# cvxgrp/DNLP

Measured on NVIDIA B200. Metric: oracle evals/s (f, grad f, g, J, Hess L), higher is better.
Workload: dtype f64

## Files before the change

dnlp_b200/_cabi.py:

```python
import ctypes as C
import os

import numpy as np

from . import tape as T

_PKG = os.path.dirname(os.path.abspath(__file__))
LIB_PATH = os.path.join(_PKG, "libdnlp_b200.so")

PROG_IDS = {"f": 0, "grad": 1, "g": 2, "jac": 3, "hess": 4, "all": 5}
NPROG = 6

c_i64p = C.POINTER(C.c_int64)
c_i32p = C.POINTER(C.c_int32)
c_f64p = C.POINTER(C.c_double)
c_f32p = C.POINTER(C.c_float)


class InstrDesc(C.Structure):
    _fields_ = [
        ("kind", C.c_int32), ("dst_space", C.c_int32), ("dst_off", C.c_int64), ("count", C.c_int64),
        ("fcode", C.c_int32), ("a_stride", C.c_int32), ("b_stride", C.c_int32), ("accumulate", C.c_int32),
        ("param", C.c_double), ("a_off", C.c_int64), ("b_off", C.c_int64),
        ("ptr", c_i64p), ("coef", c_f64p), ("f1", c_i32p), ("f2", c_i32p), ("pos", c_i32p),
        ("nterms", C.c_int64), ("row_len", C.c_int32), ("uses_lam", C.c_int32),
        ("level", C.c_int32), ("dep_mask", C.c_int32),
        ("Q", c_f64p), ("ncols", C.c_int64), ("x_off", C.c_int64), ("alpha", C.c_double),
        ("s_slot", C.c_int64),
        ("deps", c_i32p), ("n_deps", C.c_int64),
        ("dst_stride", C.c_int32), ("reserved0", C.c_int32), ("post_scale", C.c_double), ("qpos", c_i32p),
    ]


class TapeDesc(C.Structure):
    _fields_ = [
        ("n", C.c_int64), ("m", C.c_int64), ("nslots", C.c_int64), ("nnz_jac", C.c_int64), ("nnz_hess", C.c_int64),
        ("n_instr", C.c_int32), ("instrs", C.POINTER(InstrDesc)),
        ("prog", c_i32p * NPROG), ("prog_len", C.c_int32 * NPROG),
        ("f_const", C.c_double), ("grad_const", c_f64p), ("g_const", c_f64p),
        ("jac_const", c_f64p), ("hess_const", c_f64p),
        ("n_params", C.c_int64), ("params", c_f64p),
    ]


EXPORTS = [
    "dnlp_device_count", "dnlp_version", "dnlp_device_synchronize", "dnlp_create", "dnlp_destroy", "dnlp_last_error",
    "dnlp_eval_f", "dnlp_eval_grad", "dnlp_eval_g", "dnlp_eval_jac", "dnlp_eval_hess", "dnlp_eval_all",
    "dnlp_host_alloc", "dnlp_host_free", "dnlp_upload_point", "dnlp_run_device", "dnlp_profile_instrs",
    "dnlp_read_output", "dnlp_kernel_launches", "dnlp_set_cache", "dnlp_set_graphs", "dnlp_set_parallel", "dnlp_set_windows", "dnlp_set_dynamic", "dnlp_eval_dyn", "dnlp_bind_outputs", "dnlp_set_params", "dnlp_instr_kernel", "dnlp_run", "dnlp_output_ptr",
    "dnlp_batch_create", "dnlp_batch_destroy", "dnlp_batch_last_error", "dnlp_batch_eval", "dnlp_batch_upload",
    "dnlp_batch_run_device", "dnlp_batch_read_output", "dnlp_batch_profile_instrs", "dnlp_batch_kernel_launches", "dnlp_batch_profile_groups",
    "dnlp_batch_kkt_setup", "dnlp_batch_kkt_solve", "dnlp_batch_kkt_matrix",
    "dnlp_comm_unique_id", "dnlp_comm_create", "dnlp_comm_destroy", "dnlp_comm_last_error", "dnlp_comm_has_nccl",
    "dnlp_comm_ipc_handle", "dnlp_comm_open_peers", "dnlp_comm_allreduce_host",
    "dnlp_shard_create", "dnlp_shard_destroy", "dnlp_shard_last_error", "dnlp_shard_set_output",
    "dnlp_shard_root_handles", "dnlp_shard_open_root", "dnlp_shard_eval", "dnlp_shard_run_device", "dnlp_shard_set_layout",
    "dnlp_shard_share_control", "dnlp_shard_share_output", "dnlp_shard_share_unlink", "dnlp_shard_share_release", "dnlp_shard_share_reset",
    "dnlp_shard_share_inputs", "dnlp_shard_post_command", "dnlp_shard_wait_command",
]

_lib = None


def lib():
    global _lib
    if _lib is not None:
        return _lib
    if not os.path.exists(LIB_PATH):
        raise RuntimeError(
            "dnlp_b200: %s is missing - build it with `python -m dnlp_b200.build` "
            "(there is no CPU fallback for the oracle)" % LIB_PATH)
    L = C.CDLL(LIB_PATH)
    vp = C.c_void_p
    L.dnlp_device_count.restype = C.c_int
    L.dnlp_version.restype = C.c_char_p
    L.dnlp_device_synchronize.argtypes = [C.c_int]
    L.dnlp_create.argtypes = [C.POINTER(TapeDesc), C.c_int, C.POINTER(vp)]
    L.dnlp_destroy.argtypes = [vp]
    L.dnlp_destroy.restype = None
    L.dnlp_last_error.argtypes = [vp]
    L.dnlp_last_error.restype = C.c_char_p
    L.dnlp_eval_f.argtypes = [vp, c_f64p, c_f64p]
    L.dnlp_eval_grad.argtypes = [vp, c_f64p, c_f64p]
    L.dnlp_eval_g.argtypes = [vp, c_f64p, c_f64p]
    L.dnlp_eval_jac.argtypes = [vp, c_f64p, c_f64p]
    L.dnlp_eval_hess.argtypes = [vp, c_f64p, c_f64p, C.c_double, c_f64p]
    L.dnlp_eval_all.argtypes = [vp, c_f64p, c_f64p, C.c_double] + [c_f64p] * 5
    L.dnlp_host_alloc.argtypes = [C.c_int64]
    L.dnlp_host_alloc.restype = vp
    L.dnlp_host_free.argtypes = [vp]
    L.dnlp_host_free.restype = None
    L.dnlp_upload_point.argtypes = [vp, c_f64p, c_f64p, C.c_double]
    L.dnlp_run_device.argtypes = [vp, C.c_int32, C.c_int32, c_f32p]
    L.dnlp_profile_instrs.argtypes = [vp, C.c_int32, C.c_int32, c_f32p]
    L.dnlp_read_output.argtypes = [vp, C.c_int32, c_f64p]
    L.dnlp_kernel_launches.argtypes = [vp]
    L.dnlp_kernel_launches.restype = C.c_int64
    L.dnlp_set_cache.argtypes = [vp, C.c_int32]
    L.dnlp_set_graphs.argtypes = [vp, C.c_int32]
    L.dnlp_set_parallel.argtypes = [vp, C.c_int32]
    L.dnlp_set_windows.argtypes = [vp, C.c_int32]
    L.dnlp_run.argtypes = [vp, C.c_int32, c_f64p, c_f64p, C.c_double]
    L.dnlp_output_ptr.argtypes = [vp, C.c_int32]
    L.dnlp_output_ptr.restype = vp
    L.dnlp_instr_kernel.argtypes = [vp, C.c_int32]
    L.dnlp_instr_kernel.restype = C.c_char_p
    L.dnlp_set_params.argtypes = [vp, c_f64p, C.c_int64]
    L.dnlp_bind_outputs.argtypes = [vp, c_f64p, c_f64p, c_f64p, c_f64p, C.c_int32]
    L.dnlp_set_dynamic.argtypes = [vp, C.c_int32, c_i32p, C.c_int64]
    L.dnlp_eval_dyn.argtypes = [vp, C.c_int32, c_f64p, c_f64p, C.c_double, c_f64p]
    L.dnlp_batch_create.argtypes = [C.POINTER(TapeDesc), C.c_int, C.c_int32, C.POINTER(vp)]
    L.dnlp_batch_destroy.argtypes = [vp]
    L.dnlp_batch_destroy.restype = None
    L.dnlp_batch_last_error.argtypes = [vp]
    L.dnlp_batch_last_error.restype = C.c_char_p
    L.dnlp_batch_eval.argtypes = [vp] + [c_f64p] * 8
    L.dnlp_batch_upload.argtypes = [vp, c_f64p, c_f64p, c_f64p]
    L.dnlp_batch_run_device.argtypes = [vp, C.c_int32, C.c_int32, c_f32p]
    L.dnlp_batch_read_output.argtypes = [vp, C.c_int32, c_f64p]
    L.dnlp_batch_profile_instrs.argtypes = [vp, C.c_int32, C.c_int32, c_f32p]
    L.dnlp_batch_profile_groups.argtypes = [vp, C.c_int32, c_f32p, c_f64p, C.c_int32]
    L.dnlp_batch_kernel_launches.argtypes = [vp]
    L.dnlp_batch_kernel_launches.restype = C.c_int64
    L.dnlp_batch_kkt_setup.argtypes = [vp, C.c_int64] + [c_i32p] * 5
    L.dnlp_batch_kkt_solve.argtypes = [vp, C.c_int32, c_i32p] + [c_f64p] * 5 + [c_i32p, c_f64p, c_f32p]
    L.dnlp_batch_kkt_matrix.argtypes = [vp, C.c_int32, c_f64p]
    cp = C.c_char_p
    L.dnlp_comm_unique_id.argtypes = [cp]
    L.dnlp_comm_create.argtypes = [cp, C.c_int, C.c_int, C.c_int, C.POINTER(vp)]
    L.dnlp_comm_destroy.argtypes = [vp]
    L.dnlp_comm_destroy.restype = None
    L.dnlp_comm_last_error.argtypes = [vp]
    L.dnlp_comm_last_error.restype = C.c_char_p
    L.dnlp_comm_has_nccl.argtypes = [vp]
    L.dnlp_comm_ipc_handle.argtypes = [vp, cp]
    L.dnlp_comm_open_peers.argtypes = [vp, cp]
    L.dnlp_comm_allreduce_host.argtypes = [vp, c_f64p, C.c_int64]
    L.dnlp_shard_create.argtypes = [vp, vp, C.c_int, C.POINTER(vp)]
    L.dnlp_shard_destroy.argtypes = [vp]
    L.dnlp_shard_destroy.restype = None
    L.dnlp_shard_last_error.argtypes = [vp]
    L.dnlp_shard_last_error.restype = C.c_char_p
    L.dnlp_shard_set_output.argtypes = [vp, C.c_int32, C.c_int64, c_i32p, c_i32p, C.c_int64, c_i32p, c_i32p,
                                        C.c_int64, c_f64p, C.c_int64, c_i32p]
    L.dnlp_shard_root_handles.argtypes = [vp, cp]
    L.dnlp_shard_open_root.argtypes = [vp, cp]
    L.dnlp_shard_set_layout.argtypes = [vp, C.c_int32, c_i64p, c_i64p, C.c_int32, c_i64p, c_i64p]
    L.dnlp_shard_eval.argtypes = [vp, C.c_int32, c_f64p, c_f64p, C.c_double, c_f64p]
    L.dnlp_shard_run_device.argtypes = [vp, C.c_int32, C.c_int32, c_f32p]
    L.dnlp_shard_share_control.argtypes = [vp, C.c_char_p, C.c_int32]
    L.dnlp_shard_share_output.argtypes = [vp, C.c_int32, C.c_char_p, C.c_int32, C.c_int64, c_i64p, c_i64p, c_i64p,
                                          C.POINTER(c_f64p)]
    L.dnlp_shard_share_unlink.argtypes = [C.c_char_p]
    L.dnlp_shard_share_release.argtypes = [C.c_void_p, C.c_int64]
    L.dnlp_shard_share_reset.argtypes = [vp]
    L.dnlp_shard_share_inputs.argtypes = [vp, C.c_char_p, C.c_char_p, C.c_int32, C.c_int64, C.c_int64,
                                          C.POINTER(c_f64p), C.POINTER(c_f64p)]
    L.dnlp_shard_post_command.argtypes = [vp, C.c_int32, c_f64p, c_f64p, C.c_double, C.c_int32, C.POINTER(C.c_int32)]
    L.dnlp_shard_wait_command.argtypes = [vp, C.c_double, C.POINTER(C.c_int32), C.POINTER(C.c_double),
                                          C.POINTER(C.c_int32)]
    _lib = L
    return L


def device_count():
    return int(lib().dnlp_device_count())


def device_synchronize(device=0):
    if lib().dnlp_device_synchronize(int(device)) != 0:
        raise RuntimeError("dnlp_b200: cudaDeviceSynchronize failed on device %d" % device)


def _p(arr, typ):
    return None if arr is None else arr.ctypes.data_as(typ)


def f64(a):
    return np.ascontiguousarray(a, dtype=np.float64)


def pinned_empty(count):
    L = lib()
    nbytes = max(int(count), 1) * 8
    ptr = L.dnlp_host_alloc(nbytes)
    if not ptr:
        raise MemoryError("cudaMallocHost(%d) failed" % nbytes)
    buf = (C.c_double * max(int(count), 1)).from_address(ptr)
    handle = _PinnedHandle(ptr)
    buf._dnlp_handle = handle
    arr = np.frombuffer(buf, dtype=np.float64, count=int(count))
    return arr, handle


def shared_view(addr, count):
    buf = (C.c_double * max(int(count), 1)).from_address(addr)
    buf._dnlp_handle = _SharedHandle(addr, int(count))
    return np.frombuffer(buf, dtype=np.float64, count=int(count))


class _SharedHandle:
    def __init__(self, addr, count):
        self.addr, self.count = addr, count

    def __del__(self):
        try:
            if self.addr:
                lib().dnlp_shard_share_release(self.addr, self.count)
                self.addr = None
        except Exception:
            pass


class _PinnedHandle:
    def __init__(self, ptr):
        self.ptr = ptr

    def free(self):
        """Kept for API compatibility: release happens when the last array view is collected."""

    def __del__(self):
        try:
            if self.ptr:
                lib().dnlp_host_free(self.ptr)
                self.ptr = None
        except Exception:
            pass


def make_tape_desc(tape):
    keep = []
    n_instr = len(tape.instrs)
    i32max = int(np.iinfo(np.int32).max)
    for what, v in (("value slots", tape.nslots), ("Jacobian entries", tape.jac_rows.size),
                    ("Hessian entries", tape.hess_rows.size)):
        if int(v) > i32max:
            raise OverflowError("dnlp_b200: %d %s exceed the int32 index range of the device tape" % (int(v), what))
    arr = (InstrDesc * max(n_instr, 1))()
    for i, ins in enumerate(tape.instrs):
        d = arr[i]
        d.kind, d.dst_space, d.dst_off, d.count = ins.kind, ins.dst_space, int(ins.dst_off), int(ins.count)
        d.fcode, d.a_stride, d.b_stride = int(ins.fcode), int(ins.a_stride), int(ins.b_stride)
        d.accumulate = int(bool(ins.accumulate))
        d.param, d.a_off, d.b_off = float(ins.param), int(ins.a_off), int(ins.b_off)
        d.uses_lam = int(bool(ins.uses_lam))
        d.level = int(ins.level)
        d.dep_mask = int(ins.dep_mask)
        d.alpha, d.ncols, d.x_off, d.s_slot = float(ins.alpha), int(ins.ncols), int(ins.x_off), int(ins.s_slot)
        d.dst_stride, d.post_scale = int(ins.dst_stride), float(ins.post_scale)
        if ins.kind == T.K_SPMVJ:
            qpos = np.ascontiguousarray(ins.qpos, dtype=np.int32)
            keep.append(qpos)
            d.qpos = _p(qpos, c_i32p)
        if ins.kind in (T.K_POLY, T.K_SPMVJ):
            lens = np.diff(ins.ptr)
            uniform = lens.size > 0 and bool(np.all(lens == lens[0])) and lens[0] >= 1
            coef = f64(ins.coef)
            f1 = np.ascontiguousarray(ins.f1, dtype=np.int32)
            has_f2 = bool(np.any(ins.f2 >= 0))
            f2 = np.ascontiguousarray(ins.f2, dtype=np.int32) if has_f2 else None
            ptr = None if uniform else np.ascontiguousarray(ins.ptr, dtype=np.int64)
            keep += [coef, f1, f2, ptr]
            d.ptr, d.coef, d.f1, d.f2 = _p(ptr, c_i64p), _p(coef, c_f64p), _p(f1, c_i32p), _p(f2, c_i32p)
            d.nterms = int(coef.size)
            d.row_len = int(lens[0]) if uniform else 0
        elif ins.kind == T.K_GEMV:
            Q = f64(ins.Q)
            keep.append(Q)
            d.Q = _p(Q, c_f64p)
        elif ins.kind == T.K_SCALE:
            coef = f64(ins.coef)
            keep.append(coef)
            d.coef = _p(coef, c_f64p)
        if len(ins.deps):
            deps = np.ascontiguousarray(sorted(ins.deps), dtype=np.int32)
            keep.append(deps)
            d.deps, d.n_deps = _p(deps, c_i32p), int(deps.size)
        if ins.pos is not None:
            pos = np.ascontiguousarray(ins.pos, dtype=np.int32)
            keep.append(pos)
            d.pos = _p(pos, c_i32p)
    td = TapeDesc()
    td.n, td.m, td.nslots = tape.n, tape.m, tape.nslots
    td.nnz_jac, td.nnz_hess = int(tape.jac_rows.size), int(tape.hess_rows.size)
    td.n_instr, td.instrs = n_instr, arr
    for name, pid in PROG_IDS.items():
        p = np.ascontiguousarray(tape.programs.get(name, []), dtype=np.int32)
        keep.append(p)
        td.prog[pid] = _p(p, c_i32p) if p.size else None
        td.prog_len[pid] = int(p.size)
    consts = [f64(tape.grad_const), f64(tape.g_const), f64(tape.jac_const), f64(tape.hess_const)]
    keep += consts
    td.f_const = float(tape.f_const)
    td.grad_const, td.g_const, td.jac_const, td.hess_const = [_p(c, c_f64p) if c.size else None for c in consts]
    pv = f64(getattr(tape, "param_values", np.zeros(0)))
    keep.append(pv)
    td.n_params = int(getattr(tape, "n_params", 0))
    if pv.size != td.n_params:
        raise ValueError("tape has %d parameter slots but %d values" % (td.n_params, pv.size))
    td.params = _p(pv, c_f64p) if pv.size else None
    keep += [arr, td]
    return td, keep


def _require_device(L):
    if L.dnlp_device_count() <= 0:
        raise RuntimeError("dnlp_b200: no CUDA device visible (the oracle has no CPU fallback)")


class DeviceTape:

    def __init__(self, tape, device=0):
        L = lib()
        _require_device(L)
        self.tape = tape
        td, keep = make_tape_desc(tape)
        h = C.c_void_p()
        if L.dnlp_create(C.byref(td), int(device), C.byref(h)) != 0:
            raise RuntimeError("dnlp_create failed: %s" % L.dnlp_last_error(None).decode())
        self.h = h
        self._L = L

    def check(self, rc):
        if rc != 0:
            if not self.h:
                raise RuntimeError("dnlp_b200: oracle closed")
            raise RuntimeError("dnlp_b200: %s" % self._L.dnlp_last_error(self.h).decode())

    def set_params(self, values):
        self.check(self._L.dnlp_set_params(self.h, values.ctypes.data_as(c_f64p), int(values.size)))

    def bind_outputs(self, f, grad, g, jac, eager):
        p = lambda a: a.ctypes.data_as(c_f64p)
        self.check(self._L.dnlp_bind_outputs(self.h, p(f), p(grad), p(g), p(jac), int(bool(eager))))

    def close(self):
        if getattr(self, "h", None):
            self._L.dnlp_destroy(self.h)
            self.h = None

    def __del__(self):
        try:
            self.close()
        except Exception:
            pass


class DeviceBatch:

    def __init__(self, tape, batch, device=0):
        L = lib()
        _require_device(L)
        self.tape, self.batch = tape, int(batch)
        td, keep = make_tape_desc(tape)
        h = C.c_void_p()
        if L.dnlp_batch_create(C.byref(td), int(device), int(batch), C.byref(h)) != 0:
            raise RuntimeError("dnlp_batch_create failed: %s" % L.dnlp_batch_last_error(None).decode())
        self.h = h
        self._L = L

    def check(self, rc):
        if rc != 0:
            if not self.h:
                raise RuntimeError("dnlp_b200: oracle closed")
            raise RuntimeError("dnlp_b200: %s" % self._L.dnlp_batch_last_error(self.h).decode())

    def close(self):
        if getattr(self, "h", None):
            self._L.dnlp_batch_destroy(self.h)
            self.h = None

    def __del__(self):
        try:
            self.close()
        except Exception:
            pass
```

dnlp_b200/csrc/dnlp_cabi.cu:

```cuda
#include "dnlp_engine.h"

#include <algorithm>
#include <cstdio>
#include <cstdlib>
#include <cstring>
#include <string>
#include <thread>
#include <unordered_map>
#include <vector>

namespace {
thread_local std::string g_create_error;
}

namespace {

using namespace dnlp;

template <int F, bool B>
void launch_elem_t(const dnlp_oracle *o, const dnlp_instr_desc &d, int grid) {
  elem_kernel<F, B><<<grid, 256, 0, o->cur>>>(o->V, d.a_off, d.a_stride, d.b_off, d.b_stride,
                                                d.dst_off, d.count, d.param, d.dst_stride > 0 ? d.dst_stride : 1,
                                                d.post_scale);
}

bool launch_elem(const dnlp_oracle *o, const dnlp_instr_desc &d, int grid) {
  switch (d.fcode) {
#define U(F) case F: launch_elem_t<F, false>(o, d, grid); return true;
#define Bn(F) case F: launch_elem_t<F, true>(o, d, grid); return true;
    U(F_EXP) U(F_LOG) U(F_ENTR) U(F_NEG_LOG_M1) U(F_RECIP) U(F_NEG_RECIP) U(F_NEG_RECIP_SQ)
    U(F_LOGISTIC) U(F_LOGISTIC_D1) U(F_LOGISTIC_D2) U(F_POW)
    U(F_SIN) U(F_COS) U(F_NEG_SIN) U(F_NEG_COS) U(F_TAN) U(F_TAN_D1) U(F_TAN_D2)
    U(F_SINH) U(F_COSH) U(F_TANH) U(F_TANH_D1) U(F_TANH_D2)
    U(F_ASINH) U(F_ASINH_D1) U(F_ASINH_D2) U(F_ATANH) U(F_ATANH_D1) U(F_ATANH_D2)
    U(F_XEXP) U(F_XEXP_D1) U(F_XEXP_D2)
    Bn(F_REL_ENTR) Bn(F_LOG_RATIO_P1) Bn(F_DIV) Bn(F_DIV_SQ) Bn(F_DIV_CUBE)
#undef U
#undef Bn
    default: return false;
  }
}

template <int G>
void launch_poly_g(const dnlp_oracle *o, const DevInstr &I, double *dst, int grid) {
  const dnlp_instr_desc &d = I.d;
  const bool uni = d.ptr == nullptr;
#define LP(H, Un)                                                                                   \
  poly_rows_kernel<G, 2, H, Un><<<grid, 256, 0, o->cur>>>(o->V, dst, d.ptr, d.row_len, d.coef,   \
                                                             d.f1, d.f2, d.pos, d.count, d.accumulate)
  if (I.has_f2) { if (uni) LP(true, true); else LP(true, false); }
  else { if (uni) LP(false, true); else LP(false, false); }
#undef LP
}

void choose_window(const int32_t *f1, const int32_t *f2, int64_t nterms, int64_t nslots, int *w0, int *W) {
  *w0 = -1; *W = 0;
  constexpr int BK = 256;
  const int64_t nb = nslots / BK + 1;
  std::vector<int64_t> cnt((size_t)nb + 1, 0);
  int64_t total = 0;
  for (int64_t t = 0; t < nterms; ++t) {
    if (f1[t] >= 0) { ++cnt[f1[t] / BK]; ++total; }
    if (f2 && f2[t] >= 0) { ++cnt[f2[t] / BK]; ++total; }
  }
  if (total == 0) return;
  const int widths[3] = {17, 33, 65};
  int64_t best[3], at[3];
  for (int w = 0; w < 3; ++w) {
    const int64_t Wb = widths[w] < nb ? widths[w] : nb;
    int64_t run = 0;
    for (int64_t b = 0; b < Wb; ++b) run += cnt[b];
    best[w] = run; at[w] = 0;
    for (int64_t b = Wb; b < nb; ++b) {
      run += cnt[b] - cnt[b - Wb];
      if (run > best[w]) { best[w] = run; at[w] = b - Wb + 1; }
    }
  }
  if (2 * best[2] < total) return;
  for (int w = 0; w < 3; ++w) {
    if (10 * best[w] >= 9 * best[2]) {
      const int64_t Wb = widths[w] < nb ? widths[w] : nb;
      int64_t lo = at[w] * BK, hi = lo + Wb * BK;
      if (hi > nslots) hi = nslots;
      *w0 = (int)lo; *W = (int)(hi - lo);
      return;
    }
  }
}

}

int dnlp_oracle::launch(DevInstr &I) {
  const dnlp_instr_desc &d = I.d;
  if (d.count <= 0) return 0;
  double *dst = (d.dst_space == DNLP_DST_V) ? V + d.dst_off : out[d.dst_space] + d.dst_off;
  if (cur == nullptr) { cur = stream; cur_lane = 0; }
  switch (d.kind) {
    case DNLP_ELEM: {
      int grid = grid_for((d.count + 1) / 2, 1);
      if (!launch_elem(this, d, grid)) { err = "unknown elementwise function code"; return 1; }
      if (I.kname.empty()) I.kname = "elem_kernel<" + std::to_string(d.fcode) + ", " + (d.fcode >= 40 ? "1" : "0") + ">";
      break;
    }
    case DNLP_POLY: {
      if (I.contig && I.const_coef && d.count == 1 && d.nterms >= 2048 && !d.pos) {
        int64_t blocks = (d.nterms + 256 * 4 - 1) / (256 * 4);
        int64_t cap = (int64_t)sm_count * 4;
        int grid = (int)(blocks < cap ? blocks : cap);
        if (I.has_f2)
          sum_range_kernel<true><<<grid, 256, 0, cur>>>(V, dst, I.s0, I.s1, d.nterms, I.c0, d.accumulate, scratch + cur_lane * 4096, ticket + cur_lane * 16);
        else
          sum_range_kernel<false><<<grid, 256, 0, cur>>>(V, dst, I.s0, I.s1, d.nterms, I.c0, d.accumulate, scratch + cur_lane * 4096, ticket + cur_lane * 16);
        if (I.kname.empty()) I.kname = std::string("sum_range_kernel<") + (I.has_f2 ? "1" : "0") + ">";
        break;
      }
      if (I.contig && d.ptr == nullptr && d.row_len == 1 && !d.pos && !d.accumulate && d.count >= 4096) {
        int grid = grid_for(d.count, 1);
        if (I.has_f2)
          poly1_contig_kernel<true><<<grid, 256, 0, cur>>>(V, dst, d.coef, I.s0, I.s1, d.count);
        else
          poly1_contig_kernel<false><<<grid, 256, 0, cur>>>(V, dst, d.coef, I.s0, I.s1, d.count);
        if (I.kname.empty()) I.kname = std::string("poly1_contig_kernel<") + (I.has_f2 ? "1" : "0") + ">";
        break;
      }
      if (d.count == 1 && d.nterms >= 2048 && !d.pos) {
        int64_t blocks = (d.nterms + 256 * 4 - 1) / (256 * 4);
        int64_t cap = (int64_t)sm_count * 4;
        int grid = (int)(blocks < cap ? blocks : cap);
        if (I.has_f2)
          poly_reduce_kernel<true><<<grid, 256, 0, cur>>>(V, dst, d.coef, d.f1, d.f2, d.nterms, d.accumulate, scratch + cur_lane * 4096, ticket + cur_lane * 16);
        else
          poly_reduce_kernel<false><<<grid, 256, 0, cur>>>(V, dst, d.coef, d.f1, d.f2, d.nterms, d.accumulate, scratch + cur_lane * 4096, ticket + cur_lane * 16);
        if (I.kname.empty()) I.kname = std::string("poly_reduce_kernel<") + (I.has_f2 ? "1" : "0") + ">";
        break;
      }
      if (d.ptr == nullptr && d.row_len == 1) {
        int grid = grid_for((d.count + 3) / 4, 1);
        if (grid > sm_count * poly1_grid_mult) grid = sm_count * poly1_grid_mult;
        if (I.has_f2)
          poly1_stream_kernel<4, true><<<grid, 256, 0, cur>>>(V, dst, d.coef, d.f1, d.f2, d.pos, d.count, d.accumulate);
        else
          poly1_stream_kernel<4, false><<<grid, 256, 0, cur>>>(V, dst, d.coef, d.f1, d.f2, d.pos, d.count, d.accumulate);
        if (I.kname.empty()) I.kname = std::string("poly1_stream_kernel<4, ") + (I.has_f2 ? "1" : "0") + ">";
        break;
      }
      if (I.flat && flat_enabled) {
        const bool win = I.winW > 0 && win_enabled && I.winW <= 33 * 256;
        const size_t smem = win ? (size_t)I.winW * sizeof(double) : 0;
        const int per_sm = smem > 36 * 1024 ? 2 : 4;
        const int64_t nchunks = I.nchunks;
        const int64_t need = (nchunks + dnlp::FLAT_WARPS - 1) / dnlp::FLAT_WARPS;
        const int grid = (int)(need < (int64_t)sm_count * per_sm ? need : (int64_t)sm_count * per_sm);
#define LF(H, Wn, Pd)                                                                                      \
        poly_flat_kernel<H, Wn, Pd><<<grid, 256, smem, cur>>>(V, dst, d.ptr, d.row_len, d.coef, d.f1, d.f2,    \
                                                              d.pos, d.nterms, d.accumulate, I.chunk_row0,    \
                                                              I.chunk_term0, nchunks, I.win0,                 \
                                                              win ? I.winW : 0, I.pad_shift)
        const bool pad = I.pad_shift < 31;
        if (I.has_f2) {
          if (win) { if (pad) LF(true, true, true); else LF(true, true, false); }
          else { if (pad) LF(true, false, true); else LF(true, false, false); }
        } else {
          if (win) { if (pad) LF(false, true, true); else LF(false, true, false); }
          else { if (pad) LF(false, false, true); else LF(false, false, false); }
        }
#undef LF
        if (I.kname.empty())
          I.kname = std::string("poly_flat_kernel<") + (I.has_f2 ? "1" : "0") + ", " + (win ? "1" : "0") + ", " +
                    (pad ? "1" : "0") + ">";
        break;
      }
      int G = 1;
      while (G < 32 && (double)(2 * G) <= 0.8 * I.mean_len) G <<= 1;
      int grid = grid_for((d.count + 1) / 2, G);
      switch (G) {
        case 1: launch_poly_g<1>(this, I, dst, grid); break;
        case 2: launch_poly_g<2>(this, I, dst, grid); break;
        case 4: launch_poly_g<4>(this, I, dst, grid); break;
        case 8: launch_poly_g<8>(this, I, dst, grid); break;
        case 16: launch_poly_g<16>(this, I, dst, grid); break;
        default: launch_poly_g<32>(this, I, dst, grid); break;
      }
      if (I.kname.empty())
        I.kname = "poly_rows_kernel<" + std::to_string(G) + ", 2, " + (I.has_f2 ? "1" : "0") + ", " +
                  (d.ptr == nullptr ? "1" : "0") + ">";
      break;
    }
    case DNLP_SPMVJ: {
      double *jac = out[DNLP_DST_JAC];
      if (I.flat && flat_enabled) {
        const int64_t need = (I.nchunks + dnlp::FLAT_WARPS - 1) / dnlp::FLAT_WARPS;
        const int grid = (int)(need < (int64_t)sm_count * 3 ? need : (int64_t)sm_count * 3);
        if (I.pad_shift < 31)
          spmvj_flat_kernel<true><<<grid, 256, 0, cur>>>(V, dst, jac, d.ptr, d.row_len, d.coef, d.f1, I.jrank, I.jsorted, d.pos,
                                                         d.nterms, I.chunk_row0, I.chunk_term0, I.nchunks, I.pad_shift);
        else
          spmvj_flat_kernel<false><<<grid, 256, 0, cur>>>(V, dst, jac, d.ptr, d.row_len, d.coef, d.f1, I.jrank, I.jsorted, d.pos,
                                                          d.nterms, I.chunk_row0, I.chunk_term0, I.nchunks, I.pad_shift);
        if (I.kname.empty()) I.kname = std::string("spmvj_flat_kernel<") + (I.pad_shift < 31 ? "1" : "0") + ">";
      } else {
        spmvj_rows_kernel<<<grid_for(d.count, 1), 256, 0, cur>>>(V, dst, jac, d.ptr, d.row_len, d.coef, d.f1, d.qpos, d.pos, d.count);
        if (I.kname.empty()) I.kname = "spmvj_rows_kernel";
      }
      break;
    }
    case DNLP_GEMV: {
      size_t smem = (size_t)d.ncols * sizeof(double);
      if ((d.ncols & 1) == 0 && smem <= 96 * 1024) {
        int64_t cap = (int64_t)sm_count * 2;
        int grid = (int)(d.count < cap ? d.count : cap);
        gemv_cta_kernel<4, 16><<<grid, 512, smem, cur>>>(d.Q, V, d.x_off, dst, d.count, d.ncols, d.alpha);
        if (I.kname.empty()) I.kname = "gemv_cta_kernel<4, 16>";
      } else {
        int in_smem = smem <= 96 * 1024 ? 1 : 0;
        if (!in_smem) smem = 0;
        int64_t blocks = (d.count + 7) / 8;
        int64_t cap = (int64_t)sm_count * (in_smem && smem > 48 * 1024 ? 2 : 4);
        int grid = (int)(blocks < cap ? (blocks < 1 ? 1 : blocks) : cap);
        dnlp_gemv_rows_kernel<8><<<grid, 256, smem, cur>>>(d.Q, V, d.x_off, dst, d.count, d.ncols, d.alpha, in_smem);
        if (I.kname.empty()) I.kname = "dnlp_gemv_rows_kernel<8>";
      }
      break;
    }
    case DNLP_SCALE: {
      int grid = grid_for((d.count + 1) / 2, 1);
      if (!d.pos && !d.accumulate && ((reinterpret_cast<uintptr_t>(d.coef) | reinterpret_cast<uintptr_t>(dst)) & 15) == 0)
        { scale_stream_kernel<4><<<sm_count * 16, 256, 0, cur>>>(V, d.s_slot, d.coef, dst, d.count);
          if (I.kname.empty()) I.kname = "scale_stream_kernel<4>"; }
      else
        scale_kernel<<<grid, 256, 0, cur>>>(V, d.s_slot, d.coef, dst, d.pos, d.count, d.accumulate);
      break;
    }
    default:
      err = "unknown instruction kind";
      return 1;
  }
  ++launches;
  cudaError_t e = cudaPeekAtLastError();
  if (e != cudaSuccess) {
    err = std::string("kernel launch failed: ") + cudaGetErrorString(e);
    return 1;
  }
  return 0;
}

int dnlp_oracle::build_batches() {
  for (int bi = 0; bi < 2 * DNLP_NPROG; ++bi) {
    const int p = bi >> 1;
    const bool want_short = (bi & 1) != 0;
    ElemBatch &B = batch[bi];
    std::vector<dnlp::ElemDesc> descs;
    for (int32_t id : prog[p]) {
      const dnlp_instr_desc &d = instrs[id].d;
      if (d.kind != DNLP_ELEM || d.level != 0 || d.uses_lam || d.dst_space != DNLP_DST_V || d.count <= 0) continue;
      if ((d.count < batch_split) != want_short) continue;
      bool merged = false;
      for (auto &e : descs) {
        if (e.nout < 3 && e.a_off == d.a_off && e.b_off == d.b_off && e.count == d.count &&
            e.a_stride == d.a_stride && e.b_stride == d.b_stride) {
          e.fcode[e.nout] = d.fcode; e.param[e.nout] = d.param; e.dst_off[e.nout] = d.dst_off;
          e.dst_stride[e.nout] = d.dst_stride > 0 ? d.dst_stride : 1; e.scale[e.nout] = d.post_scale; ++e.nout;
          merged = true;
          break;
        }
      }
      if (!merged) {
        dnlp::ElemDesc e{};
        e.a_off = d.a_off; e.b_off = d.b_off; e.count = d.count; e.a_stride = d.a_stride; e.b_stride = d.b_stride;
        e.nout = 1; e.fcode[0] = d.fcode; e.param[0] = d.param; e.dst_off[0] = d.dst_off;
        e.dst_stride[0] = d.dst_stride > 0 ? d.dst_stride : 1; e.scale[0] = d.post_scale;
        for (int k = 1; k < 3; ++k) { e.dst_stride[k] = 1; e.scale[k] = 1.0; }
        descs.push_back(e);
      }
      B.members.push_back(id);
    }
    if (B.members.size() < 2) { B.members.clear(); continue; }
    for (auto &e : descs) {
      e.group = dnlp::GRP_NONE;
      if (e.nout < 2 || !fuse_enabled) continue;
      const int fam = dnlp::elem_family(e.fcode[0]);
      bool same = fam != dnlp::GRP_NONE;
      for (int k = 1; k < e.nout; ++k) same = same && dnlp::elem_family(e.fcode[k]) == fam;
      if (same) e.group = fam;
    }
    int64_t tiles = 0;
    for (auto &e : descs) { e.tile0 = tiles; tiles += (e.count + dnlp::ELEM_TILE - 1) / dnlp::ELEM_TILE; }
    B.ndesc = (int)descs.size();
    B.total_tiles = tiles;
    if (upload(descs.data(), (int64_t)descs.size(), &B.descs)) return 1;
  }
  return 0;
}

int dnlp_oracle::launch_node(int32_t node) {
  if (node >= 0) return launch(instrs[node]);
  ElemBatch &B = batch[-node - 1];
  if (cur == nullptr) { cur = stream; cur_lane = 0; }
  int64_t cap = (int64_t)sm_count * 8;
  int grid = (int)(B.total_tiles < cap ? B.total_tiles : cap);
  dnlp::elem_batch_kernel<<<grid, 256, 0, cur>>>(V, B.descs, B.ndesc, B.total_tiles);
  ++launches;
  cudaError_t e = cudaPeekAtLastError();
  if (e != cudaSuccess) { err = std::string("kernel launch failed: ") + cudaGetErrorString(e); return 1; }
  return 0;
}

int dnlp_oracle::issue_serial(const std::vector<int32_t> &nodes) {
  cur = stream; cur_lane = 0;
  for (int32_t nd : nodes) if (launch_node(nd)) return 1;
  return 0;
}

cudaEvent_t dnlp_oracle::event_at(size_t i) {
  while (ev_pool.size() <= i) {
    cudaEvent_t e = nullptr;
    if (cudaEventCreateWithFlags(&e, cudaEventDisableTiming) != cudaSuccess) return nullptr;
    ev_pool.push_back(e);
  }
  return ev_pool[i];
}

int dnlp_oracle::issue_parallel(const std::vector<int32_t> &nodes) {
  const size_t N = nodes.size();
  if (N < 2 || !parallel_enabled) return issue_serial(nodes);
  std::unordered_map<int32_t, int> producer;
  for (size_t k = 0; k < N; ++k) {
    if (nodes[k] >= 0) producer[nodes[k]] = (int)k;
    else for (int32_t id : batch[-nodes[k] - 1].members) producer[id] = (int)k;
  }
  std::vector<int> lane_of(N, 0);
  int last_on_lane[NLANE];
  bool joined[NLANE];
  for (int l = 0; l < NLANE; ++l) { last_on_lane[l] = -1; joined[l] = (l == 0); }
  int last_writer[6] = {-1, -1, -1, -1, -1, -1};
  int rr = 0;
  cudaEvent_t fork = event_at(0);
  if (!fork) { err = "cudaEventCreate failed"; return 1; }
  CK(cudaEventRecord(fork, stream));
  std::vector<int> deps;
  for (size_t k = 0; k < N; ++k) {
    deps.clear();
    if (nodes[k] >= 0) {
      const DevInstr &I = instrs[nodes[k]];
      for (int32_t d : I.deps) {
        auto it = producer.find(d);
        if (it != producer.end() && it->second < (int)k) deps.push_back(it->second);
      }
      if (I.d.dst_space != DNLP_DST_V) {
        if (last_writer[I.d.dst_space] >= 0) deps.push_back(last_writer[I.d.dst_space]);
        last_writer[I.d.dst_space] = (int)k;
      }
      if (I.d.kind == DNLP_SPMVJ) {
        if (last_writer[DNLP_DST_JAC] >= 0) deps.push_back(last_writer[DNLP_DST_JAC]);
        last_writer[DNLP_DST_JAC] = (int)k;
      }
    }
    int L = -1;
    if (nodes[k] >= 0 && big_serial_terms > 0 && instrs[nodes[k]].d.kind != DNLP_ELEM &&
        instrs[nodes[k]].d.nterms >= big_serial_terms) L = 0;
    if (L < 0) for (int d : deps) if (last_on_lane[lane_of[d]] == d && !(big_serial_terms > 0 && lane_of[d] == 0)) { L = lane_of[d]; break; }
    if (L < 0) for (int l = big_serial_terms > 0 ? 1 : 0; l < NLANE; ++l) if (last_on_lane[l] < 0) { L = l; break; }
    if (L < 0) { L = big_serial_terms > 0 ? 1 + rr % (NLANE - 1) : rr; rr = (rr + 1) % NLANE; }
    if (!joined[L]) { CK(cudaStreamWaitEvent(lane[L], fork, 0)); joined[L] = true; }
    for (int d : deps)
      if (lane_of[d] != L) CK(cudaStreamWaitEvent(lane[L], event_at(1 + (size_t)d), 0));
    cur = lane[L]; cur_lane = L;
    const int rc = launch_node(nodes[k]);
    cur = stream; cur_lane = 0;
    if (rc) return 1;
    cudaEvent_t done = event_at(1 + k);
    if (!done) { err = "cudaEventCreate failed"; return 1; }
    CK(cudaEventRecord(done, lane[L]));
    lane_of[k] = L;
    last_on_lane[L] = (int)k;
  }
  for (int l = 1; l < NLANE; ++l)
    if (joined[l] && last_on_lane[l] >= 0) CK(cudaStreamWaitEvent(stream, event_at(1 + (size_t)last_on_lane[l]), 0));
  return 0;
}

int dnlp_oracle::run_programs(const int *progs, int nprogs, bool force) {
  std::vector<int32_t> nodes;
  std::vector<uint8_t> done(valid);
  if (force || !cache_enabled) std::fill(done.begin(), done.end(), 0);
  uint64_t key = 1469598103934665603ull;
  for (int q = 0; q < nprogs; ++q) {
    const int p = progs[q];
    for (int bi = 2 * p + 1; bi >= 2 * p; --bi) {
      ElemBatch &B = batch[bi];
      bool use_batch = !B.members.empty();
      if (use_batch) for (int32_t id : B.members) if (done[id]) { use_batch = false; break; }
      if (use_batch) {
        nodes.push_back(-(bi + 1));
        key = (key ^ (uint64_t)(0x10000 + bi)) * 1099511628211ull;
        for (int32_t id : B.members) done[id] = 2;
      }
    }
    for (int32_t id : prog[p]) {
      const DevInstr &I = instrs[id];
      const bool keep = cacheable(I);
      if (done[id] == 2) continue;
      if (keep && done[id]) continue;
      nodes.push_back(id);
      key = (key ^ (uint64_t)(id + 1)) * 1099511628211ull;
      if (keep) done[id] = 1;
    }
    for (auto &f : done) if (f == 2) f = 1;
  }
  if (nodes.empty()) return 0;

  if (capturing) {
    if (issue_parallel(nodes)) return 1;
  } else if (graphs_enabled && nodes.size() >= 2) {
    auto it = graphs.find(key);
    if (it != graphs.end()) {
      const GraphEntry &ge = it->second;
      if (ge.plan == nodes) {
        CK(cudaGraphLaunch(ge.exec, stream));
        launches += ge.nlaunch;
      } else if (issue_serial(nodes)) return 1;
    } else if (graphs.size() < 64) {
      const int64_t before = launches;
      capturing = true;
      CK(cudaStreamBeginCapture(stream, cudaStreamCaptureModeThreadLocal));
      const int rc = issue_parallel(nodes);
      cudaGraph_t g = nullptr;
      cudaError_t ce = cudaStreamEndCapture(stream, &g);
      capturing = false;
      if (rc) { if (g) cudaGraphDestroy(g); cudaGetLastError(); return 1; }
      if (ce != cudaSuccess) { err = std::string("graph capture failed: ") + cudaGetErrorString(ce); return 1; }
      GraphEntry ge;
      ge.plan = nodes;
      ge.nlaunch = launches - before;
      CK(cudaGraphInstantiate(&ge.exec, g, 0));
      cudaGraphDestroy(g);
      graphs.emplace(key, ge);
      CK(cudaGraphLaunch(ge.exec, stream));
    } else if (issue_serial(nodes)) return 1;
  } else if (issue_serial(nodes)) return 1;

  for (int32_t nd : nodes) {
    if (nd < 0) { for (int32_t id : batch[-nd - 1].members) valid[id] = 1; continue; }
    if (cacheable(instrs[nd])) valid[nd] = 1;
  }
  return 0;
}

static int stage_threads() { return dnlp_stage_threads(); }
int dnlp_stage_threads() {
  static const int T = [] {
    unsigned hw = std::thread::hardware_concurrency();
    int ranks = 1;
    if (const char *e = getenv("LOCAL_WORLD_SIZE")) ranks = atoi(e) > 0 ? atoi(e) : 1;
    if (const char *e = getenv("DNLP_STAGE_THREADS")) return atoi(e) > 0 ? atoi(e) : 1;
    int t = (int)(hw / (unsigned)ranks) - (ranks > 1 ? 1 : 2);
    return t < 1 ? 1 : (t > 14 ? 14 : t);
  }();
  return T;
}

static bool stage_point(double *dst, const double *src, int64_t n, bool have_old) {
  const size_t bytes = (size_t)n * sizeof(double);
  auto work = [&](int64_t lo, int64_t hi, bool *changed) {
    const size_t b = (size_t)(hi - lo) * sizeof(double);
    if (have_old && memcmp(dst + lo, src + lo, b) == 0) { *changed = false; return; }
    memcpy(dst + lo, src + lo, b);
    *changed = true;
  };
  if (bytes < (4u << 20)) {
    bool ch = true;
    work(0, n, &ch);
    return ch;
  }
  const int T = stage_threads();
  const int64_t chunk = (n + T - 1) / T;
  int any = 0;
#pragma omp parallel for num_threads(T) schedule(static, 1) reduction(| : any)
  for (int t = 0; t < T; ++t) {
    const int64_t lo = t * chunk, hi = lo + chunk < n ? lo + chunk : n;
    if (lo < hi) {
      bool ch = true;
      work(lo, hi, &ch);
      any |= ch ? 1 : 0;
    }
  }
  return any != 0;
}

static bool same_as_mirror(const double *mir, const double *src, int64_t n) {
  const size_t bytes = (size_t)n * sizeof(double);
  if (bytes < (1u << 20)) return memcmp(mir, src, bytes) == 0;
  const int T = stage_threads();
  const int64_t chunk = (n + T - 1) / T;
  int diff = 0;
#pragma omp parallel for num_threads(T) schedule(static, 1) reduction(| : diff)
  for (int t = 0; t < T; ++t) {
    const int64_t lo = t * chunk, hi = lo + chunk < n ? lo + chunk : n;
    if (lo < hi && memcmp(mir + lo, src + lo, (size_t)(hi - lo) * sizeof(double)) != 0) diff |= 1;
  }
  return diff == 0;
}

static int stage_and_upload(double *hmir, double *dev, const double *src, int64_t count, bool have_old,
                            cudaStream_t stream, bool *changed, std::string &err) {
  *changed = false;
  if (have_old && count > 0 && same_as_mirror(hmir, src, count)) return 0;
  constexpr int64_t PIECE = (4 << 20) / sizeof(double);
  for (int64_t lo = 0; lo < count; lo += PIECE) {
    const int64_t len = count - lo < PIECE ? count - lo : PIECE;
    if (stage_point(hmir + lo, src + lo, len, have_old)) {
      CK(cudaMemcpyAsync(dev + lo, hmir + lo, (size_t)len * sizeof(double), cudaMemcpyHostToDevice, stream));
      *changed = true;
    }
  }
  return 0;
}

int dnlp_oracle::put_x(const double *x) {
  bool changed = false;
  if (stage_and_upload(hx, V, x, n, have_last_x && cache_enabled, stream, &changed, err)) return 1;
  if (!changed && have_last_x && cache_enabled) return 0;
  invalidate(1);
  have_last_x = true;
  ++x_epoch;
  return 0;
}

int dnlp_oracle::put_lam(const double *lam, double sigma) {
  if (!have_last_lam || hlam[0] != sigma) {
    invalidate(2);
    hlam[0] = sigma;
    CK(cudaMemcpyAsync(V + n, hlam, sizeof(double), cudaMemcpyHostToDevice, stream));
  }
  if (m > 0 && lam != nullptr) {
    bool lam_changed = false;
    if (stage_and_upload(hlam + 1, V + n + 1, lam, m, have_last_lam, stream, &lam_changed, err)) return 1;
    if (lam_changed) invalidate(4);
  }
  have_last_lam = true;
  return 0;
}

int dnlp_oracle::put_x_runs(const double *xg, const std::vector<int64_t> &src, const std::vector<int64_t> &len) {
  bool any = false;
  int64_t off = 0;
  for (size_t r = 0; r < src.size(); ++r) {
    bool ch = false;
    if (stage_and_upload(hx + off, V + off, xg + src[r], len[r], have_last_x && cache_enabled, stream, &ch, err)) return 1;
    any = any || ch;
    off += len[r];
  }
  if (off != n) { err = "variable runs do not cover the local point"; return 1; }
  if (!any && have_last_x && cache_enabled) return 0;
  invalidate(1);
  have_last_x = true;
  ++x_epoch;
  return 0;
}

int dnlp_oracle::put_lam_runs(const double *lg, double sigma, const std::vector<int64_t> &src, const std::vector<int64_t> &len) {
  if (!have_last_lam || hlam[0] != sigma) {
    invalidate(2);
    hlam[0] = sigma;
    CK(cudaMemcpyAsync(V + n, hlam, sizeof(double), cudaMemcpyHostToDevice, stream));
  }
  int64_t off = 0;
  bool any = false;
  if (lg == nullptr) { have_last_lam = true; return 0; }
  for (size_t r = 0; r < src.size(); ++r) {
    bool ch = false;
    if (stage_and_upload(hlam + 1 + off, V + n + 1 + off, lg + src[r], len[r], have_last_lam, stream, &ch, err)) return 1;
    any = any || ch;
    off += len[r];
  }
  if (off != m) { err = "constraint runs do not cover the local multipliers"; return 1; }
  if (any) invalidate(4);
  have_last_lam = true;
  return 0;
}

int dnlp_oracle::fetch(int space, double *host) {
  if (host == nullptr || out_len[space] == 0) return 0;
  CK(cudaMemcpyAsync(host, out[space], (size_t)out_len[space] * sizeof(double), cudaMemcpyDeviceToHost, stream));
  return 0;
}

int dnlp_oracle::launch_eager() {
  CK(cudaStreamWaitEvent(stream, ev_copied, 0));
  const int progs[4] = {DNLP_PROG_F, DNLP_PROG_GRAD, DNLP_PROG_G, DNLP_PROG_JAC};
  if (run_programs(progs, 4, false)) return 1;
  for (int s = DNLP_DST_GRAD; s <= DNLP_DST_JAC; ++s)
    if (bound[s] && dyn_len[s] > 0) {
      dnlp::gather_kernel<<<grid_for(dyn_len[s], 1), 256, 0, stream>>>(out[s], dyn_pos[s], dyn_buf[s], dyn_len[s]);
      ++launches;
    }
  CK(cudaEventRecord(ev_ready, stream));
  CK(cudaStreamWaitEvent(cstream, ev_ready, 0));
  for (int s = DNLP_DST_F; s <= DNLP_DST_JAC; ++s) {
    if (!bound[s]) continue;
    const bool dyn = s != DNLP_DST_F && dyn_len[s] > 0;
    const int64_t cnt = dyn ? dyn_len[s] : out_len[s];
    if (cnt > 0)
      CK(cudaMemcpyAsync(bound[s], dyn ? dyn_buf[s] : out[s], (size_t)cnt * sizeof(double), cudaMemcpyDeviceToHost, cstream));
    CK(cudaEventRecord(ev_out[s], cstream));
  }
  CK(cudaEventRecord(ev_copied, cstream));
  eager_epoch = x_epoch;
  return 0;
}

int dnlp_oracle::deliver(int space, int prog, double *host_out) {
  if (eager && cache_enabled && host_out != nullptr && bound[space] == host_out) {
    if (eager_epoch != x_epoch && launch_eager()) return 1;
    CK(cudaEventSynchronize(ev_out[space]));
    return 0;
  }
  if (eager) CK(cudaStreamWaitEvent(stream, ev_copied, 0));
  if (run_program(prog, false)) return 1;
  if (fetch(space, host_out)) return 1;
  CK(cudaStreamSynchronize(stream));
  return 0;
}

extern "C" {

int dnlp_device_count(void) {
  int c = 0;
  if (cudaGetDeviceCount(&c) != cudaSuccess) { cudaGetLastError(); return 0; }
  return c;
}

const char *dnlp_version(void) { return "dnlp_b200 0.2 (sm_100a)"; }

int dnlp_device_synchronize(int device) {
  if (cudaSetDevice(device) != cudaSuccess || cudaDeviceSynchronize() != cudaSuccess) { cudaGetLastError(); return 1; }
  return 0;
}

const char *dnlp_last_error(dnlp_oracle *o) { return o ? o->err.c_str() : g_create_error.c_str(); }

void dnlp_destroy(dnlp_oracle *o) {
  if (!o) return;
  cudaSetDevice(o->device);
  if (o->stream) cudaStreamSynchronize(o->stream);
  for (auto &kv : o->graphs) if (kv.second.exec) cudaGraphExecDestroy(kv.second.exec);
  for (void *p : o->owned) cudaFree(p);
  if (o->hx) cudaFreeHost(o->hx);
  if (o->hlam) cudaFreeHost(o->hlam);
  if (o->cstream) cudaStreamSynchronize(o->cstream);
  if (o->ev0) cudaEventDestroy(o->ev0);
  if (o->ev1) cudaEventDestroy(o->ev1);
  if (o->ev_ready) cudaEventDestroy(o->ev_ready);
  if (o->ev_copied) cudaEventDestroy(o->ev_copied);
  for (int s2 = 0; s2 < 6; ++s2) if (o->ev_out[s2]) cudaEventDestroy(o->ev_out[s2]);
  if (o->cstream) cudaStreamDestroy(o->cstream);
  for (cudaEvent_t e : o->ev_pool) cudaEventDestroy(e);
  for (int l = 1; l < dnlp_oracle::NLANE; ++l) if (o->lane[l]) cudaStreamDestroy(o->lane[l]);
  if (o->stream) cudaStreamDestroy(o->stream);
  delete o;
}

static int create_impl(dnlp_oracle *o, const dnlp_tape_desc *t) {
  std::string &err = o->err;
  CK(cudaSetDevice(o->device));
  cudaDeviceProp prop;
  CK(cudaGetDeviceProperties(&prop, o->device));
  o->sm_count = prop.multiProcessorCount;
  CK(cudaStreamCreateWithFlags(&o->stream, cudaStreamNonBlocking));
  CK(cudaEventCreate(&o->ev0));
  CK(cudaEventCreate(&o->ev1));
  CK(cudaStreamCreateWithFlags(&o->cstream, cudaStreamNonBlocking));
  CK(cudaEventCreateWithFlags(&o->ev_ready, cudaEventDisableTiming));
  CK(cudaEventCreateWithFlags(&o->ev_copied, cudaEventDisableTiming));
  for (int s2 = 0; s2 < 6; ++s2) CK(cudaEventCreateWithFlags(&o->ev_out[s2], cudaEventDisableTiming));
  o->n = t->n; o->m = t->m; o->nslots = t->nslots; o->nnz_jac = t->nnz_jac; o->nnz_hess = t->nnz_hess;
  o->n_params = t->n_params;
  if (t->n_params < 0 || t->n + 1 + t->m + t->n_params > t->nslots) { err = "parameter slots exceed the value buffer"; return 1; }
  if (const char *e = getenv("DNLP_WIN_MIN_TERMS")) o->win_min_terms = atoll(e);
  if (const char *e = getenv("DNLP_NO_SIGMA_CACHE")) o->sigma_cache_enabled = atoi(e) == 0;
  if (const char *e = getenv("DNLP_BATCH_SPLIT")) o->batch_split = atoll(e);
  if (const char *e = getenv("DNLP_FLAT_MIN_TERMS")) o->flat_min_terms = atoll(e);
  if (const char *e = getenv("DNLP_NO_FLAT")) o->flat_enabled = atoi(e) == 0;
  if (const char *e = getenv("DNLP_POLY1_GRID_MULT")) o->poly1_grid_mult = atoi(e) > 0 ? atoi(e) : 4;
  if (const char *e = getenv("DNLP_WINDOWS")) o->win_enabled = atoi(e) != 0;
  if (const char *e = getenv("DNLP_NO_WINDOWS")) o->win_enabled = atoi(e) == 0 && o->win_enabled;
  if (const char *e = getenv("DNLP_NO_ELEM_FUSION")) o->fuse_enabled = atoi(e) == 0;
  if (const char *e = getenv("DNLP_NO_PARALLEL")) o->parallel_enabled = atoi(e) == 0;
  if (const char *e = getenv("DNLP_BIG_SERIAL_TERMS")) o->big_serial_terms = atoll(e);

  void *p = nullptr;
  CK(cudaMalloc(&p, (size_t)(t->nslots + 2) * sizeof(double)));
  o->owned.push_back(p);
  o->V = static_cast<double *>(p);
  CK(cudaMemset(o->V, 0, (size_t)(t->nslots + 2) * sizeof(double)));
  if (t->n_params > 0 && t->params)
    CK(cudaMemcpy(o->V + t->n + 1 + t->m, t->params, (size_t)t->n_params * sizeof(double), cudaMemcpyHostToDevice));

  CK(cudaMallocHost(&p, (size_t)(t->n + 2) * sizeof(double)));
  o->hx = static_cast<double *>(p);
  CK(cudaMallocHost(&p, (size_t)(t->m + 2) * sizeof(double)));
  o->hlam = static_cast<double *>(p);
  CK(cudaMalloc(&p, (size_t)dnlp_oracle::NLANE * 4096 * sizeof(double)));
  o->owned.push_back(p);
  o->scratch = static_cast<double *>(p);
  CK(cudaMalloc(&p, (size_t)dnlp_oracle::NLANE * 16 * sizeof(unsigned int)));
  o->owned.push_back(p);
  o->ticket = static_cast<unsigned int *>(p);
  CK(cudaMemset(o->ticket, 0, (size_t)dnlp_oracle::NLANE * 16 * sizeof(unsigned int)));
  o->lane[0] = o->stream;
  for (int l = 1; l < dnlp_oracle::NLANE; ++l) CK(cudaStreamCreateWithFlags(&o->lane[l], cudaStreamNonBlocking));
  o->cur = o->stream;

  const int64_t lens[6] = {0, 1, t->n, t->m, t->nnz_jac, t->nnz_hess};
  const double *consts[6] = {nullptr, &t->f_const, t->grad_const, t->g_const, t->jac_const, t->hess_const};
  for (int s = 1; s < 6; ++s) {
    o->out_len[s] = lens[s];
    CK(cudaMalloc(&p, (size_t)(lens[s] + 2) * sizeof(double)));
    o->owned.push_back(p);
    o->out[s] = static_cast<double *>(p);
    if (lens[s] > 0) {
      if (consts[s])
        CK(cudaMemcpy(o->out[s], consts[s], (size_t)lens[s] * sizeof(double), cudaMemcpyHostToDevice));
      else
        CK(cudaMemset(o->out[s], 0, (size_t)lens[s] * sizeof(double)));
    }
  }

  o->instrs.resize(t->n_instr);
  o->valid.assign(t->n_instr, 0);
  for (int i = 0; i < t->n_instr; ++i) {
    const dnlp_instr_desc &h = t->instrs[i];
    DevInstr &D = o->instrs[i];
    D.d = h;
    D.d.ptr = nullptr; D.d.coef = nullptr; D.d.f1 = nullptr; D.d.f2 = nullptr; D.d.pos = nullptr; D.d.Q = nullptr;
    D.d.deps = nullptr;
    D.d.qpos = nullptr;
    if (D.d.dst_stride <= 0) D.d.dst_stride = 1;
    if (h.kind == DNLP_ELEM && D.d.post_scale == 0.0 && h.post_scale == 0.0) D.d.post_scale = 1.0;
    for (int64_t k = 0; k < h.n_deps; ++k) {
      if (h.deps[k] < 0 || h.deps[k] >= i) { err = "instruction depends on a later or unknown instruction"; return 1; }
      D.deps.push_back(h.deps[k]);
    }
    if (h.kind == DNLP_POLY || h.kind == DNLP_SPMVJ) {
      if (h.ptr) { if (o->upload(h.ptr, h.count + 1, const_cast<int64_t **>(&D.d.ptr))) return 1; }
      if (o->upload(h.coef, h.nterms, const_cast<double **>(&D.d.coef))) return 1;
      if (o->upload(h.f1, h.nterms, const_cast<int32_t **>(&D.d.f1))) return 1;
      if (h.f2) { if (o->upload(h.f2, h.nterms, const_cast<int32_t **>(&D.d.f2))) return 1; }
      if (h.kind == DNLP_SPMVJ) {
        if (h.f2 || !h.qpos) { err = "SPMVJ needs single-factor terms and Jacobian positions"; return 1; }
        for (int64_t t2 = 0; t2 < h.nterms; ++t2) {
          if (h.f1[t2] >= 0 && ((h.f1[t2] & 1) || h.f1[t2] + 1 >= t->nslots)) { err = "SPMVJ: value slots must be even (pair layout)"; return 1; }
          if (h.qpos[t2] >= t->nnz_jac) { err = "SPMVJ: Jacobian position out of range"; return 1; }
        }
        if (o->upload(h.qpos, h.nterms, const_cast<int32_t **>(&D.d.qpos))) return 1;
      }
      D.has_f2 = h.f2 != nullptr;
      D.mean_len = h.count > 0 ? (double)h.nterms / (double)h.count : 1.0;
      if (h.kind == DNLP_POLY && h.nterms >= 2048 && (h.count == 1 || (!h.ptr && h.row_len == 1)) && h.f1[0] >= 0 &&
          (!h.f2 || h.f2[0] >= 0)) {
        bool contig = true, cc = true;
        for (int64_t t2 = 1; t2 < h.nterms && contig; ++t2) {
          if (h.f1[t2] != h.f1[0] + t2) contig = false;
          else if (h.f2 && h.f2[t2] != h.f2[0] + t2) contig = false;
          if (h.coef[t2] != h.coef[0]) cc = false;
        }
        D.contig = contig;
        D.const_coef = contig && cc;
        D.s0 = h.f1[0];
        D.s1 = h.f2 ? h.f2[0] : 0;
        D.c0 = h.coef[0];
      }
      if (h.nterms >= o->flat_min_terms && h.count >= 2 && !(h.ptr == nullptr && h.row_len == 1) &&
          D.mean_len <= 64.0 && h.count < ((int64_t)1 << 31) - 1) {
        auto rb = [&](int64_t r) -> int64_t { return h.ptr ? h.ptr[r] : r * (int64_t)h.row_len; };
        std::vector<int32_t> row0;
        std::vector<int64_t> term0;
        bool ok = true;
        int64_t R = 0;
        while (R < h.count) {
          const int64_t a0 = rb(R) & ~(int64_t)1;
          int64_t Rn = R;
          while (Rn < h.count && rb(Rn + 1) <= a0 + dnlp::FLAT_CHUNK) ++Rn;
          if (Rn == R) { ok = false; break; }
          row0.push_back((int32_t)R);
          term0.push_back(a0);
          R = Rn;
        }
        if (ok) {
          row0.push_back((int32_t)h.count);
          D.nchunks = (int64_t)term0.size();
          if (o->upload(row0.data(), (int64_t)row0.size(), &D.chunk_row0)) return 1;
          if (o->upload(term0.data(), (int64_t)term0.size(), &D.chunk_term0)) return 1;
          const int64_t L = (int64_t)(D.mean_len + 0.5) > 0 ? (int64_t)(D.mean_len + 0.5) : 1;
          int best_conf = 1 << 30;
          const int shifts[3] = {31, 4, 5};
          for (int si = 0; si < 3; ++si) {
            int hits[16] = {0};
            int conf = 0;
            for (int j = 0; j < 16; ++j) {
              const int64_t k = j * L;
              const int64_t q = k + (shifts[si] >= 31 ? 0 : ((k >> shifts[si]) << 1));
              conf = std::max(conf, ++hits[q & 15]);
            }
            if (conf < best_conf) { best_conf = conf; D.pad_shift = shifts[si]; }
          }
          D.flat = true;
          if (h.kind == DNLP_SPMVJ) {
            std::vector<uint8_t> jrank((size_t)h.nterms + 2, 0);
            std::vector<int32_t> jsorted((size_t)h.nterms + 2, -1);
            const int64_t nch = D.nchunks;
#pragma omp parallel for schedule(static)
            for (int64_t ci = 0; ci < nch; ++ci) {
              const int64_t t0c = rb(row0[ci]), t1c = rb(row0[ci + 1]);
              const int nown = (int)(t1c - t0c);
              int idx[dnlp::FLAT_CHUNK];
              for (int i = 0; i < nown; ++i) idx[i] = i;
              std::sort(idx, idx + nown, [&](int a, int b) {
                const int32_t qa = h.qpos[t0c + a], qb = h.qpos[t0c + b];
                const uint32_t ua = qa < 0 ? 0xFFFFFFFFu : (uint32_t)qa, ub = qb < 0 ? 0xFFFFFFFFu : (uint32_t)qb;
                return ua != ub ? ua < ub : a < b;
              });
              for (int i = 0; i < nown; ++i) {
                jrank[t0c + idx[i]] = (uint8_t)i;
                jsorted[t0c + i] = h.qpos[t0c + idx[i]];
              }
            }
            if (o->upload(jrank.data(), (int64_t)jrank.size(), &D.jrank)) return 1;
            if (o->upload(jsorted.data(), (int64_t)jsorted.size(), &D.jsorted)) return 1;
          }
        }
      }
      if (D.flat && h.nterms >= o->win_min_terms)
        choose_window(h.f1, h.f2, h.nterms, t->nslots, &D.win0, &D.winW);
    } else if (h.kind == DNLP_GEMV) {
      if (o->upload(h.Q, h.count * h.ncols, const_cast<double **>(&D.d.Q))) return 1;
    } else if (h.kind == DNLP_SCALE) {
      if (o->upload(h.coef, h.count, const_cast<double **>(&D.d.coef))) return 1;
    }
    if ((h.kind == DNLP_POLY || h.kind == DNLP_SCALE || h.kind == DNLP_SPMVJ) && h.pos) {
      if (o->upload(h.pos, h.count, const_cast<int32_t **>(&D.d.pos))) return 1;
    }
  }
  for (const DevInstr &D : o->instrs)
    if (D.d.accumulate && D.d.dst_space >= 1 && D.d.dst_space <= 5) o->space_has_acc[D.d.dst_space] = true;
  for (int q = 0; q < DNLP_NPROG; ++q) {
    o->prog[q].assign(t->prog[q], t->prog[q] + t->prog_len[q]);
    for (int32_t id : o->prog[q])
      if (id < 0 || id >= t->n_instr) { err = "program references an unknown instruction"; return 1; }
  }
  if (o->build_batches()) return 1;
  CK(cudaFuncSetAttribute(dnlp::dnlp_gemv_rows_kernel<8>, cudaFuncAttributeMaxDynamicSharedMemorySize, 96 * 1024));
  CK(cudaFuncSetAttribute(dnlp::gemv_cta_kernel<4, 16>, cudaFuncAttributeMaxDynamicSharedMemorySize, 96 * 1024));
#define FA(H, Pd)                                                                                                       \
  CK(cudaFuncSetAttribute(dnlp::poly_flat_kernel<H, true, Pd>, cudaFuncAttributeMaxDynamicSharedMemorySize, 72 * 1024)); \
  CK(cudaFuncSetAttribute(dnlp::poly_flat_kernel<H, true, Pd>, cudaFuncAttributePreferredSharedMemoryCarveout, 100))
  FA(true, true); FA(true, false); FA(false, true); FA(false, false);
#undef FA
  CK(cudaStreamSynchronize(o->stream));
  return 0;
}

int dnlp_create(const dnlp_tape_desc *t, int device, dnlp_oracle **out) {
  *out = nullptr;
  dnlp_oracle *o = new dnlp_oracle();
  o->device = device;
  if (create_impl(o, t)) {
    g_create_error = o->err;
    dnlp_destroy(o);
    return 1;
  }
  *out = o;
  return 0;
}

#define ENTER(o)                                   \
  if ((o) == nullptr) { g_create_error = "oracle handle is NULL (closed or never created)"; return 1; } \
  std::string &err = (o)->err;                     \
  CK(cudaSetDevice((o)->device))

int dnlp_eval_f(dnlp_oracle *o, const double *x, double *f) {
  ENTER(o);
  if (o->put_x(x) || o->deliver(DNLP_DST_F, DNLP_PROG_F, f)) return 1;
  return 0;
}

int dnlp_eval_grad(dnlp_oracle *o, const double *x, double *grad) {
  ENTER(o);
  if (o->put_x(x) || o->deliver(DNLP_DST_GRAD, DNLP_PROG_GRAD, grad)) return 1;
  return 0;
}

int dnlp_eval_g(dnlp_oracle *o, const double *x, double *g) {
  ENTER(o);
  if (o->put_x(x) || o->deliver(DNLP_DST_G, DNLP_PROG_G, g)) return 1;
  return 0;
}

int dnlp_eval_jac(dnlp_oracle *o, const double *x, double *vals) {
  ENTER(o);
  if (o->put_x(x) || o->deliver(DNLP_DST_JAC, DNLP_PROG_JAC, vals)) return 1;
  return 0;
}

int dnlp_eval_hess(dnlp_oracle *o, const double *x, const double *lam, double sigma, double *vals) {
  ENTER(o);
  if (o->put_x(x) || o->put_lam(lam, sigma) || o->run_program(DNLP_PROG_HESS, false) ||
      o->fetch(DNLP_DST_HESS, vals)) return 1;
  CK(cudaStreamSynchronize(o->stream));
  return 0;
}

int dnlp_eval_all(dnlp_oracle *o, const double *x, const double *lam, double sigma,
                  double *f, double *grad, double *g, double *jac, double *hess) {
  ENTER(o);
  if (o->eager) CK(cudaStreamWaitEvent(o->stream, o->ev_copied, 0));
  if (o->put_x(x) || o->put_lam(lam, sigma) || o->run_program(DNLP_PROG_ALL, false)) return 1;
  if (o->fetch(DNLP_DST_F, f) || o->fetch(DNLP_DST_GRAD, grad) || o->fetch(DNLP_DST_G, g) ||
      o->fetch(DNLP_DST_JAC, jac) || o->fetch(DNLP_DST_HESS, hess)) return 1;
  CK(cudaStreamSynchronize(o->stream));
  return 0;
}

int dnlp_set_params(dnlp_oracle *o, const double *values, int64_t count) {
  ENTER(o);
  if (count != o->n_params) { err = "wrong number of parameter values"; return 1; }
  if (count == 0) return 0;
  CK(cudaStreamSynchronize(o->cstream));
  CK(cudaMemcpyAsync(o->V + o->n + 1 + o->m, values, (size_t)count * sizeof(double), cudaMemcpyHostToDevice, o->stream));
  CK(cudaStreamSynchronize(o->stream));
  o->invalidate(8);
  ++o->x_epoch;
  return 0;
}

int dnlp_bind_outputs(dnlp_oracle *o, double *f, double *grad, double *g, double *jac, int32_t eager) {
  ENTER(o);
  CK(cudaStreamSynchronize(o->cstream));
  o->bound[DNLP_DST_F] = f; o->bound[DNLP_DST_GRAD] = grad; o->bound[DNLP_DST_G] = g; o->bound[DNLP_DST_JAC] = jac;
  o->eager = eager != 0;
  o->eager_epoch = ~0ull;
  return 0;
}

int dnlp_set_dynamic(dnlp_oracle *o, int32_t space, const int32_t *pos, int64_t count) {
  ENTER(o);
  if (space < DNLP_DST_GRAD || space > DNLP_DST_HESS) { err = "bad output id"; return 1; }
  for (int64_t i = 0; i < count; ++i)
    if (pos[i] < 0 || pos[i] >= o->out_len[space]) { err = "dynamic position out of range"; return 1; }
  if (o->upload(pos, count, &o->dyn_pos[space])) return 1;
  void *p = nullptr;
  CK(cudaMalloc(&p, (size_t)(count + 2) * sizeof(double)));
  o->owned.push_back(p);
  o->dyn_buf[space] = static_cast<double *>(p);
  o->dyn_len[space] = count;
  return 0;
}

int dnlp_eval_dyn(dnlp_oracle *o, int32_t prog, const double *x, const double *lam, double sigma,
                  double *compact) {
  ENTER(o);
  if (prog < DNLP_PROG_GRAD || prog > DNLP_PROG_HESS) { err = "bad program id"; return 1; }
  const int space = prog + 1;
  if (o->put_x(x)) return 1;
  if (prog != DNLP_PROG_HESS && o->eager && o->cache_enabled && compact != nullptr && o->bound[space] == compact &&
      o->dyn_len[space] > 0) {
    if (o->eager_epoch != o->x_epoch && o->launch_eager()) return 1;
    CK(cudaEventSynchronize(o->ev_out[space]));
    return 0;
  }
  if (o->eager) CK(cudaStreamWaitEvent(o->stream, o->ev_copied, 0));
  if (prog == DNLP_PROG_HESS && o->put_lam(lam, sigma)) return 1;
  if (o->run_program(prog, false)) return 1;
  const int64_t cnt = o->dyn_len[space];
  if (cnt > 0) {
    int grid = o->grid_for(cnt, 1);
    dnlp::gather_kernel<<<grid, 256, 0, o->stream>>>(o->out[space], o->dyn_pos[space], o->dyn_buf[space], cnt);
    ++o->launches;
    CK(cudaMemcpyAsync(compact, o->dyn_buf[space], (size_t)cnt * sizeof(double), cudaMemcpyDeviceToHost, o->stream));
  }
  CK(cudaStreamSynchronize(o->stream));
  return 0;
}

int dnlp_run(dnlp_oracle *o, int32_t prog, const double *x, const double *lam, double sigma) {
  ENTER(o);
  if (o->cstream) CK(cudaStreamSynchronize(o->cstream));
  if (prog < 0 || prog >= DNLP_NPROG) { err = "bad program id"; return 1; }
  if (o->put_x(x)) return 1;
  if ((prog == DNLP_PROG_HESS || prog == DNLP_PROG_ALL) && o->put_lam(lam, sigma)) return 1;
  if (o->run_program(prog, false)) return 1;
  CK(cudaStreamSynchronize(o->stream));
  return 0;
}

void *dnlp_output_ptr(dnlp_oracle *o, int32_t space) {
  if (!o) return nullptr;
  if (space < DNLP_DST_F || space > DNLP_DST_HESS) return nullptr;
  return o->out[space];
}

void *dnlp_host_alloc(int64_t bytes) {
  void *p = nullptr;
  if (cudaMallocHost(&p, (size_t)bytes) != cudaSuccess) { cudaGetLastError(); return nullptr; }
  return p;
}

void dnlp_host_free(void *p) { if (p) cudaFreeHost(p); }

int dnlp_upload_point(dnlp_oracle *o, const double *x, const double *lam, double sigma) {
  ENTER(o);
  o->have_last_x = false;
  o->have_last_lam = false;
  if (o->put_x(x)) return 1;
  if (lam != nullptr || o->m == 0) { if (o->put_lam(lam, sigma)) return 1; }
  CK(cudaStreamSynchronize(o->stream));
  return 0;
}

int dnlp_run_device(dnlp_oracle *o, int32_t prog_mask, int32_t iters, float *elapsed_ms) {
  ENTER(o);
  if (o->cstream) CK(cudaStreamSynchronize(o->cstream));
  int progs[DNLP_NPROG], nprogs = 0;
  for (int p = 0; p < DNLP_NPROG; ++p) if (prog_mask & (1 << p)) progs[nprogs++] = p;
  if ((prog_mask & 0x1F) == 0x1F) { progs[0] = DNLP_PROG_ALL; nprogs = 1; }
  auto step = [&]() -> int {
    std::fill(o->valid.begin(), o->valid.end(), 0);
    return o->run_programs(progs, nprogs, false);
  };
  cudaGraphExec_t exec = nullptr;
  int64_t per_step = 0;
  if (iters <= 0) { if (elapsed_ms) *elapsed_ms = 0.f; return 0; }
  if (o->graphs_enabled) {
    const int64_t before = o->launches;
    o->capturing = true;
    CK(cudaStreamBeginCapture(o->stream, cudaStreamCaptureModeThreadLocal));
    const int rc = step();
    cudaGraph_t g = nullptr;
    cudaError_t ce = cudaStreamEndCapture(o->stream, &g);
    o->capturing = false;
    if (rc) { if (g) cudaGraphDestroy(g); return 1; }
    if (ce != cudaSuccess) { err = std::string("graph capture failed: ") + cudaGetErrorString(ce); return 1; }
    per_step = o->launches - before;
    o->launches = before;
    CK(cudaGraphInstantiate(&exec, g, 0));
    cudaGraphDestroy(g);
  }
  CK(cudaEventRecord(o->ev0, o->stream));
  for (int it = 0; it < iters; ++it) {
    if (exec) { CK(cudaGraphLaunch(exec, o->stream)); o->launches += per_step; }
    else if (step()) return 1;
  }
  CK(cudaEventRecord(o->ev1, o->stream));
  CK(cudaEventSynchronize(o->ev1));
  float ms = 0.f;
  CK(cudaEventElapsedTime(&ms, o->ev0, o->ev1));
  if (exec) cudaGraphExecDestroy(exec);
  if (elapsed_ms) *elapsed_ms = ms;
  return 0;
}

int dnlp_profile_instrs(dnlp_oracle *o, int32_t p, int32_t iters, float *ms_per_instr) {
  ENTER(o);
  if (o->cstream) CK(cudaStreamSynchronize(o->cstream));
  if (p < 0 || p >= DNLP_NPROG) { err = "bad program id"; return 1; }
  const size_t ni = o->instrs.size();
  for (size_t i = 0; i < ni; ++i) ms_per_instr[i] = 0.f;
  for (int32_t id : o->prog[p])
    if (o->launch(o->instrs[id])) return 1;
  CK(cudaStreamSynchronize(o->stream));
  const int reps = 3;
  for (int it = 0; it < iters; ++it) {
    for (int32_t id : o->prog[p]) {
      CK(cudaEventRecord(o->ev0, o->stream));
      for (int r = 0; r < reps; ++r)
        if (o->launch(o->instrs[id])) return 1;
      CK(cudaEventRecord(o->ev1, o->stream));
      CK(cudaEventSynchronize(o->ev1));
      float ms = 0.f;
      CK(cudaEventElapsedTime(&ms, o->ev0, o->ev1));
      ms_per_instr[id] += ms / (float)(iters * reps);
    }
  }
  return 0;
}

int dnlp_read_output(dnlp_oracle *o, int32_t space, double *out) {
  ENTER(o);
  if (o->cstream) CK(cudaStreamSynchronize(o->cstream));
  if (space < 1 || space > 5) { err = "bad output id"; return 1; }
  if (o->fetch(space, out)) return 1;
  CK(cudaStreamSynchronize(o->stream));
  return 0;
}

int64_t dnlp_kernel_launches(dnlp_oracle *o) { return o ? o->launches : -1; }

const char *dnlp_instr_kernel(dnlp_oracle *o, int32_t instr) {
  if (!o) return "";
  if (instr < 0 || (size_t)instr >= o->instrs.size()) return "";
  return o->instrs[instr].kname.c_str();
}

int dnlp_set_graphs(dnlp_oracle *o, int32_t enabled) {
  if (!o) return 1;
  o->graphs_enabled = enabled != 0;
  return 0;
}

int dnlp_set_parallel(dnlp_oracle *o, int32_t enabled) {
  ENTER(o);
  CK(cudaStreamSynchronize(o->stream));
  o->parallel_enabled = enabled != 0;
  for (auto &kv : o->graphs) if (kv.second.exec) cudaGraphExecDestroy(kv.second.exec);
  o->graphs.clear();
  return 0;
}

int dnlp_set_windows(dnlp_oracle *o, int32_t enabled) {
  ENTER(o);
  CK(cudaStreamSynchronize(o->stream));
  o->win_enabled = enabled != 0;
  for (auto &kv : o->graphs) if (kv.second.exec) cudaGraphExecDestroy(kv.second.exec);
  o->graphs.clear();
  for (auto &I : o->instrs) I.kname.clear();
  return 0;
}

int dnlp_set_cache(dnlp_oracle *o, int32_t enabled) {
  if (!o) return 1;
  o->cache_enabled = enabled != 0;
  o->have_last_x = false;
  std::fill(o->valid.begin(), o->valid.end(), 0);
  return 0;
}

}
```

dnlp_b200/csrc/dnlp_engine.h:

```cpp
#pragma once
#include "../../include/dnlp_b200.h"
#include "dnlp_kernels.cuh"

#include <cstdio>
#include <cstring>
#include <string>
#include <unordered_map>
#include <vector>

int dnlp_stage_threads();

namespace dnlp_detail {

#define CK(call)                                                                           \
  do {                                                                                     \
    cudaError_t e_ = (call);                                                               \
    if (e_ != cudaSuccess) {                                                               \
      char buf_[512];                                                                      \
      snprintf(buf_, sizeof buf_, "%s failed at %s:%d: %s", #call, __FILE__, __LINE__,      \
               cudaGetErrorString(e_));                                                    \
      err = buf_;                                                                          \
      return 1;                                                                            \
    }                                                                                      \
  } while (0)

struct DevInstr {
  dnlp_instr_desc d;
  double mean_len = 1.0;
  bool has_f2 = false;
  std::string kname;
  std::vector<int32_t> deps;
  bool contig = false;
  bool const_coef = false;
  int64_t s0 = 0, s1 = 0;
  double c0 = 1.0;
  int win0 = -1, winW = 0;
  bool flat = false;
  int32_t *chunk_row0 = nullptr;
  int64_t *chunk_term0 = nullptr;
  int64_t nchunks = 0;
  int pad_shift = 31;
  uint8_t *jrank = nullptr;
  int32_t *jsorted = nullptr;
};

struct ElemBatch {
  dnlp::ElemDesc *descs = nullptr;
  int ndesc = 0;
  int64_t total_tiles = 0;
  std::vector<int32_t> members;
};

}
using dnlp_detail::DevInstr;
using dnlp_detail::ElemBatch;

struct dnlp_oracle {
  int device = 0;
  int sm_count = 148;
  int64_t n = 0, m = 0, nslots = 0, nnz_jac = 0, nnz_hess = 0, n_params = 0;
  cudaStream_t stream = nullptr;
  double *V = nullptr;
  double *out[6] = {nullptr, nullptr, nullptr, nullptr, nullptr, nullptr};
  int64_t out_len[6] = {0, 0, 0, 0, 0, 0};
  std::vector<DevInstr> instrs;
  std::vector<int32_t> prog[DNLP_NPROG];
  ElemBatch batch[2 * DNLP_NPROG];
  int64_t batch_split = 1 << 16;
  std::vector<void *> owned;
  std::vector<uint8_t> valid;
  double *hx = nullptr;
  double *hlam = nullptr;
  bool have_last_x = false;
  bool have_last_lam = false;
  bool cache_enabled = true;
  int64_t launches = 0;
  std::string err;
  cudaEvent_t ev0 = nullptr, ev1 = nullptr;
  cudaStream_t cstream = nullptr;
  cudaEvent_t ev_ready = nullptr, ev_copied = nullptr, ev_out[6] = {nullptr, nullptr, nullptr, nullptr, nullptr, nullptr};
  double *bound[6] = {nullptr, nullptr, nullptr, nullptr, nullptr, nullptr};
  bool eager = false;
  uint64_t x_epoch = 0, eager_epoch = ~0ull;
  int launch_eager();
  int deliver(int space, int prog, double *host_out);
  struct GraphEntry {
    cudaGraphExec_t exec = nullptr;
    int64_t nlaunch = 0;
    std::vector<int32_t> plan;
  };
  std::unordered_map<uint64_t, GraphEntry> graphs;
  bool graphs_enabled = true;
  bool capturing = false;
  int32_t *dyn_pos[6] = {nullptr, nullptr, nullptr, nullptr, nullptr, nullptr};
  double *dyn_buf[6] = {nullptr, nullptr, nullptr, nullptr, nullptr, nullptr};
  int64_t dyn_len[6] = {0, 0, 0, 0, 0, 0};
  double *scratch = nullptr;
  unsigned int *ticket = nullptr;
  static constexpr int NLANE = 8;
  cudaStream_t lane[NLANE] = {nullptr, nullptr, nullptr, nullptr, nullptr, nullptr, nullptr, nullptr};
  cudaStream_t cur = nullptr;
  int cur_lane = 0;
  std::vector<cudaEvent_t> ev_pool;
  bool parallel_enabled = true;
  int64_t big_serial_terms = 1 << 24;
  bool win_enabled = false;
  bool fuse_enabled = true;
  bool flat_enabled = true;
  int poly1_grid_mult = 8;
  int64_t flat_min_terms = 1 << 18;
  int64_t win_min_terms = 1 << 18;

  template <typename T>
  int upload(const T *host, int64_t count, T **dev) {
    *dev = nullptr;
    if (count <= 0 || host == nullptr) return 0;
    void *p = nullptr;
    CK(cudaMalloc(&p, (size_t)count * sizeof(T)));
    owned.push_back(p);
    CK(cudaMemcpy(p, host, (size_t)count * sizeof(T), cudaMemcpyHostToDevice));
    *dev = static_cast<T *>(p);
    return 0;
  }

  int grid_for(int64_t work_items, int threads_per_item, int block = 256) const {
    int64_t need = (work_items * threads_per_item + block - 1) / block;
    int64_t cap = (int64_t)sm_count * 8;
    if (need >= cap) return (int)cap;
    if (need < 1) need = 1;
    if (need > sm_count) need = ((need + sm_count - 1) / sm_count) * sm_count;
    return (int)need;
  }

  int launch(DevInstr &I);
  int build_batches();
  bool space_has_acc[6] = {false, false, false, false, false, false};
  bool sigma_cache_enabled = true;
  bool cacheable(const DevInstr &I) const {
    if (I.d.dst_space == DNLP_DST_V) return !I.d.uses_lam;
    return sigma_cache_enabled && I.d.dep_mask == 2 && !I.d.accumulate && !space_has_acc[I.d.dst_space];
  }
  void invalidate(int bits) {
    for (size_t i = 0; i < instrs.size(); ++i) {
      const int mk = instrs[i].d.dep_mask;
      if (mk == 0 || (mk & bits)) valid[i] = 0;
    }
  }
  int run_program(int p, bool force) { return run_programs(&p, 1, force); }
  int run_programs(const int *progs, int nprogs, bool force);
  int issue_serial(const std::vector<int32_t> &nodes);
  int issue_parallel(const std::vector<int32_t> &nodes);
  int launch_node(int32_t node);
  cudaEvent_t event_at(size_t i);
  int put_x(const double *x);
  int put_lam(const double *lam, double sigma);
  int put_x_runs(const double *xg, const std::vector<int64_t> &src, const std::vector<int64_t> &len);
  int put_lam_runs(const double *lg, double sigma, const std::vector<int64_t> &src, const std::vector<int64_t> &len);
  int fetch(int space, double *host);
};
```

dnlp_b200/csrc/dnlp_kernels.cuh:

```cuda
#pragma once
#include <cuda_runtime.h>
#include <math.h>
#include <stdint.h>

namespace dnlp {

enum : int {
  F_EXP = 1, F_LOG = 2, F_ENTR = 3, F_NEG_LOG_M1 = 4, F_RECIP = 5, F_NEG_RECIP = 6, F_NEG_RECIP_SQ = 7,
  F_LOGISTIC = 8, F_LOGISTIC_D1 = 9, F_LOGISTIC_D2 = 10, F_POW = 11,
  F_SIN = 12, F_COS = 13, F_NEG_SIN = 14, F_NEG_COS = 15, F_TAN = 16, F_TAN_D1 = 17, F_TAN_D2 = 18,
  F_SINH = 19, F_COSH = 20, F_TANH = 21, F_TANH_D1 = 22, F_TANH_D2 = 23,
  F_ASINH = 24, F_ASINH_D1 = 25, F_ASINH_D2 = 26, F_ATANH = 27, F_ATANH_D1 = 28, F_ATANH_D2 = 29,
  F_XEXP = 30, F_XEXP_D1 = 31, F_XEXP_D2 = 32,
  F_REL_ENTR = 40, F_LOG_RATIO_P1 = 41, F_DIV = 42, F_DIV_SQ = 43, F_DIV_CUBE = 44
};

template <int F>
__device__ __forceinline__ double apply_fn(double a, double b, double p) {
  if constexpr (F == F_EXP) return exp(a);
  else if constexpr (F == F_LOG) return log(a);
  else if constexpr (F == F_ENTR) {
    if (a == 0.0) return -0.0;
    double r = -(a * log(a));
    return isnan(r) ? -INFINITY : r;
  }
  else if constexpr (F == F_NEG_LOG_M1) return -log(a) - 1.0;
  else if constexpr (F == F_RECIP) return 1.0 / a;
  else if constexpr (F == F_NEG_RECIP) return -1.0 / a;
  else if constexpr (F == F_NEG_RECIP_SQ) return -1.0 / (a * a);
  else if constexpr (F == F_LOGISTIC) {
    if (isnan(a)) return a;
    return fmax(a, 0.0) + log1p(exp(-fabs(a)));
  }
  else if constexpr (F == F_LOGISTIC_D1) { double e = exp(a); return e / (1.0 + e); }
  else if constexpr (F == F_LOGISTIC_D2) { double e = exp(a); double d = e + 1.0; return e / (d * d); }
  else if constexpr (F == F_POW) {
    if (p == 2.0) return a * a;
    if (p == 1.0) return a;
    if (p == 0.0) return 1.0;
    if (p == 3.0) return a * a * a;
    if (p == 4.0) { const double q = a * a; return q * q; }
    if (p == -1.0) return 1.0 / a;
    if (p == 0.5) return a == -INFINITY ? INFINITY : sqrt(a);
    return pow(a, p);
  }
  else if constexpr (F == F_SIN) return sin(a);
  else if constexpr (F == F_COS) return cos(a);
  else if constexpr (F == F_NEG_SIN) return -sin(a);
  else if constexpr (F == F_NEG_COS) return -cos(a);
  else if constexpr (F == F_TAN) return tan(a);
  else if constexpr (F == F_TAN_D1) { double c = cos(a); return 1.0 / (c * c); }
  else if constexpr (F == F_TAN_D2) { double c = cos(a); return 2.0 * tan(a) / (c * c); }
  else if constexpr (F == F_SINH) return sinh(a);
  else if constexpr (F == F_COSH) return cosh(a);
  else if constexpr (F == F_TANH) return tanh(a);
  else if constexpr (F == F_TANH_D1) { double c = cosh(a); return 1.0 / (c * c); }
  else if constexpr (F == F_TANH_D2) { double c = cosh(a); return -2.0 * (tanh(a) / (c * c)); }
  else if constexpr (F == F_ASINH) return asinh(a);
  else if constexpr (F == F_ASINH_D1) return 1.0 / sqrt(1.0 + a * a);
  else if constexpr (F == F_ASINH_D2) return -a / pow(1.0 + a * a, 1.5);
  else if constexpr (F == F_ATANH) return atanh(a);
  else if constexpr (F == F_ATANH_D1) return 1.0 / (1.0 - a * a);
  else if constexpr (F == F_ATANH_D2) { double d = 1.0 - a * a; return 2.0 * a / (d * d); }
  else if constexpr (F == F_XEXP) return a * exp(a);
  else if constexpr (F == F_XEXP_D1) return exp(a) * (1.0 + a);
  else if constexpr (F == F_XEXP_D2) return exp(a) * (2.0 + a);
  else if constexpr (F == F_REL_ENTR) {
    if (isnan(a) || isnan(b)) return NAN;
    if (a > 0.0 && b > 0.0) return a * log(a / b);
    if (a == 0.0 && b >= 0.0) return 0.0;
    return INFINITY;
  }
  else if constexpr (F == F_LOG_RATIO_P1) return log(a / b) + 1.0;
  else if constexpr (F == F_DIV) return a / b;
  else if constexpr (F == F_DIV_SQ) return a / (b * b);
  else if constexpr (F == F_DIV_CUBE) return a / (b * b * b);
  else return NAN;
}

template <int F, bool BINARY>
__global__ void __launch_bounds__(256)
elem_kernel(double *__restrict__ V, int64_t a_off, int a_stride, int64_t b_off, int b_stride,
            int64_t dst_off, int64_t count, double p, int dst_stride, double post_scale) {
  const double *__restrict__ A = V + a_off;
  const double *__restrict__ B = V + b_off;
  double *__restrict__ D = V + dst_off;
  const int64_t tid = (int64_t)blockIdx.x * blockDim.x + threadIdx.x;
  const int64_t nthr = (int64_t)gridDim.x * blockDim.x;
  const bool vec_ok = a_stride == 1 && ((a_off | dst_off) & 1) == 0 && dst_stride == 1 &&
                      (!BINARY || b_stride == 0 || (b_stride == 1 && (b_off & 1) == 0));
  if (vec_ok) {
    const int64_t n2 = count >> 1;
    const double2 *A2 = reinterpret_cast<const double2 *>(A);
    const double2 *B2 = reinterpret_cast<const double2 *>(B);
    double2 *D2 = reinterpret_cast<double2 *>(D);
    const double b0 = BINARY && b_stride == 0 ? B[0] : 0.0;
    for (int64_t i = tid; i < n2; i += nthr) {
      double2 a = A2[i];
      double2 b = make_double2(b0, b0);
      if (BINARY && b_stride == 1) b = B2[i];
      double2 r;
      r.x = post_scale * apply_fn<F>(a.x, b.x, p);
      r.y = post_scale * apply_fn<F>(a.y, b.y, p);
      D2[i] = r;
    }
    if ((count & 1) && tid == 0) {
      int64_t k = count - 1;
      D[k] = post_scale * apply_fn<F>(A[k], BINARY ? B[k * b_stride] : 0.0, p);
    }
  } else {
    for (int64_t k = tid; k < count; k += nthr)
      D[k * dst_stride] = post_scale * apply_fn<F>(A[k * a_stride], BINARY ? B[k * b_stride] : 0.0, p);
  }
}

__device__ __forceinline__ double ld_slot(const double *__restrict__ V, int idx) {
  return idx < 0 ? 1.0 : __ldg(V + idx);
}

template <int G, bool HAS_F2, bool UNIFORM>
__global__ void __launch_bounds__(256)
poly_kernel(const double *__restrict__ V, double *__restrict__ dst, const int64_t *__restrict__ ptr,
            int row_len, const double *__restrict__ coef, const int32_t *__restrict__ f1,
            const int32_t *__restrict__ f2, const int32_t *__restrict__ pos, int64_t count,
            int accumulate) {
  const int lane = threadIdx.x & (G - 1);
  const int64_t group = ((int64_t)blockIdx.x * blockDim.x + threadIdx.x) / G;
  const int64_t ngroups = ((int64_t)gridDim.x * blockDim.x) / G;
  for (int64_t row = group; row < count; row += ngroups) {
    int64_t t0, t1;
    if (UNIFORM) { t0 = row * (int64_t)row_len; t1 = t0 + row_len; }
    else { t0 = __ldg(ptr + row); t1 = __ldg(ptr + row + 1); }
    double acc = 0.0;
    for (int64_t t = t0 + lane; t < t1; t += G) {
      double v = __ldg(coef + t) * ld_slot(V, __ldg(f1 + t));
      if (HAS_F2) v *= ld_slot(V, __ldg(f2 + t));
      acc += v;
    }
#pragma unroll
    for (int s = G >> 1; s > 0; s >>= 1) acc += __shfl_xor_sync(0xffffffffu, acc, s, G);
    if (lane == 0) {
      int64_t d = pos ? (int64_t)__ldg(pos + row) : row;
      dst[d] = accumulate ? dst[d] + acc : acc;
    }
  }
}

template <bool HAS_F2>
__global__ void __launch_bounds__(256)
poly1_kernel(const double *__restrict__ V, double *__restrict__ dst, const double *__restrict__ coef,
             const int32_t *__restrict__ f1, const int32_t *__restrict__ f2,
             const int32_t *__restrict__ pos, int64_t count, int accumulate) {
  const int64_t tid = (int64_t)blockIdx.x * blockDim.x + threadIdx.x;
  const int64_t nthr = (int64_t)gridDim.x * blockDim.x;
  for (int64_t k = tid; k < count; k += nthr) {
    double v = __ldg(coef + k) * ld_slot(V, __ldg(f1 + k));
    if (HAS_F2) v *= ld_slot(V, __ldg(f2 + k));
    int64_t d = pos ? (int64_t)__ldg(pos + k) : k;
    dst[d] = accumulate ? dst[d] + v : v;
  }
}

template <int UNROLL>
__global__ void __launch_bounds__(256)
dnlp_gemv_rows_kernel(const double *__restrict__ Q, const double *__restrict__ V, int64_t x_off,
            double *__restrict__ dst, int64_t nrows, int64_t ncols, double alpha, int x_in_smem) {
  extern __shared__ __align__(16) double xs[];
  const double *__restrict__ x = V + x_off;
  if (x_in_smem) {
    for (int64_t j = threadIdx.x; j < ncols; j += blockDim.x) xs[j] = x[j];
    __syncthreads();
    x = xs;
  }
  const int lane = threadIdx.x & 31;
  const int64_t warp = ((int64_t)blockIdx.x * blockDim.x + threadIdx.x) >> 5;
  const int64_t nwarps = ((int64_t)gridDim.x * blockDim.x) >> 5;
  const bool vec_ok = (ncols & 1) == 0 && (x_in_smem || (x_off & 1) == 0);
  for (int64_t row = warp; row < nrows; row += nwarps) {
    const double *__restrict__ q = Q + row * ncols;
    double acc = 0.0;
    if (vec_ok) {
      const double2 *q2 = reinterpret_cast<const double2 *>(q);
      const double2 *x2 = reinterpret_cast<const double2 *>(x);
      const int64_t n2 = ncols >> 1;
      int64_t j = lane;
      for (; j + (UNROLL - 1) * 32 < n2; j += UNROLL * 32) {
        double2 a[UNROLL];
#pragma unroll
        for (int u = 0; u < UNROLL; ++u) a[u] = __ldcs(q2 + j + u * 32);
#pragma unroll
        for (int u = 0; u < UNROLL; ++u) {
          double2 b = x2[j + u * 32];
          acc = fma(a[u].x, b.x, acc);
          acc = fma(a[u].y, b.y, acc);
        }
      }
      for (; j < n2; j += 32) {
        double2 a = __ldcs(q2 + j);
        double2 b = x2[j];
        acc = fma(a.x, b.x, acc);
        acc = fma(a.y, b.y, acc);
      }
    } else {
      for (int64_t j = lane; j < ncols; j += 32) acc = fma(q[j], x[j], acc);
    }
#pragma unroll
    for (int s = 16; s > 0; s >>= 1) acc += __shfl_xor_sync(0xffffffffu, acc, s);
    if (lane == 0) dst[row] = alpha * acc;
  }
}

static __global__ void __launch_bounds__(256)
scale_kernel(const double *__restrict__ V, int64_t s_slot, const double *__restrict__ coef,
             double *__restrict__ dst, const int32_t *__restrict__ pos, int64_t count, int accumulate) {
  const double s = __ldg(V + s_slot);
  const int64_t tid = (int64_t)blockIdx.x * blockDim.x + threadIdx.x;
  const int64_t nthr = (int64_t)gridDim.x * blockDim.x;
  if (!pos && !accumulate && ((reinterpret_cast<uintptr_t>(coef) | reinterpret_cast<uintptr_t>(dst)) & 15) == 0) {
    const int64_t n2 = count >> 1;
    const double2 *c2 = reinterpret_cast<const double2 *>(coef);
    double2 *d2 = reinterpret_cast<double2 *>(dst);
    for (int64_t i = tid; i < n2; i += nthr) {
      double2 c = __ldcs(c2 + i);
      __stcs(d2 + i, make_double2(s * c.x, s * c.y));
    }
    if ((count & 1) && tid == 0) dst[count - 1] = s * coef[count - 1];
  } else {
    for (int64_t k = tid; k < count; k += nthr) {
      int64_t d = pos ? (int64_t)pos[k] : k;
      double v = s * coef[k];
      dst[d] = accumulate ? dst[d] + v : v;
    }
  }
}

}

namespace dnlp {

__device__ __forceinline__ uint64_t l2_policy_evict_first() {
  uint64_t p;
  asm("createpolicy.fractional.L2::evict_first.b64 %0, 1.0;" : "=l"(p));
  return p;
}
__device__ __forceinline__ uint64_t l2_policy_evict_last() {
  uint64_t p;
  asm("createpolicy.fractional.L2::evict_last.b64 %0, 1.0;" : "=l"(p));
  return p;
}
__device__ __forceinline__ double ld_stream_f64(const double *p, uint64_t pol) {
  double v;
  asm("ld.global.nc.L1::no_allocate.L2::cache_hint.f64 %0, [%1], %2;" : "=d"(v) : "l"(p), "l"(pol));
  return v;
}
__device__ __forceinline__ int ld_stream_s32(const int32_t *p, uint64_t pol) {
  int v;
  asm("ld.global.nc.L1::no_allocate.L2::cache_hint.s32 %0, [%1], %2;" : "=r"(v) : "l"(p), "l"(pol));
  return v;
}
__device__ __forceinline__ double2 ld_stream_f64x2(const double2 *p, uint64_t pol) {
  double2 v;
  asm("ld.global.nc.L1::no_allocate.L2::cache_hint.v2.f64 {%0, %1}, [%2], %3;"
               : "=d"(v.x), "=d"(v.y) : "l"(p), "l"(pol));
  return v;
}
__device__ __forceinline__ double ld_keep_f64(const double *p, uint64_t pol) {
  double v;
  asm volatile("ld.global.L2::cache_hint.f64 %0, [%1], %2;" : "=d"(v) : "l"(p), "l"(pol) : "memory");
  return v;
}
__device__ __forceinline__ void st_stream_f64(double *p, double v, uint64_t pol) {
  asm volatile("st.global.L1::no_allocate.L2::cache_hint.f64 [%0], %1, %2;" :: "l"(p), "d"(v), "l"(pol) : "memory");
}
__device__ __forceinline__ void st_stream_f64x2(double2 *p, double2 v, uint64_t pol) {
  asm volatile("st.global.L1::no_allocate.L2::cache_hint.v2.f64 [%0], {%1, %2}, %3;"
               :: "l"(p), "d"(v.x), "d"(v.y), "l"(pol) : "memory");
}
__device__ __forceinline__ double gather_slot(const double *__restrict__ V, int idx, uint64_t pol) {
  return idx < 0 ? 1.0 : ld_keep_f64(V + idx, pol);
}

template <int U>
__global__ void __launch_bounds__(256)
scale_stream_kernel(const double *__restrict__ V, int64_t s_slot, const double *__restrict__ coef,
                    double *__restrict__ dst, int64_t count) {
  const double s = __ldg(V + s_slot);
  const uint64_t pf = l2_policy_evict_first();
  const int64_t n2 = count >> 1;
  const double2 *c2 = reinterpret_cast<const double2 *>(coef);
  double2 *d2 = reinterpret_cast<double2 *>(dst);
  const int64_t stride = (int64_t)gridDim.x * blockDim.x;
  int64_t i = (int64_t)blockIdx.x * blockDim.x + threadIdx.x;
  for (; i + (U - 1) * stride < n2; i += U * stride) {
    double2 c[U];
#pragma unroll
    for (int u = 0; u < U; ++u) c[u] = ld_stream_f64x2(c2 + i + u * stride, pf);
#pragma unroll
    for (int u = 0; u < U; ++u) st_stream_f64x2(d2 + i + u * stride, make_double2(s * c[u].x, s * c[u].y), pf);
  }
  for (; i < n2; i += stride) {
    double2 c = ld_stream_f64x2(c2 + i, pf);
    st_stream_f64x2(d2 + i, make_double2(s * c.x, s * c.y), pf);
  }
  if ((count & 1) && blockIdx.x == 0 && threadIdx.x == 0) dst[count - 1] = s * coef[count - 1];
}

template <int U, int NWARPS>
__global__ void __launch_bounds__(NWARPS * 32)
gemv_cta_kernel(const double *__restrict__ Q, const double *__restrict__ V, int64_t x_off,
                double *__restrict__ dst, int64_t nrows, int64_t ncols, double alpha) {
  extern __shared__ __align__(16) double xs[];
  __shared__ double part[2][NWARPS];
  const double *__restrict__ x = V + x_off;
  for (int64_t j = threadIdx.x; j < ncols; j += blockDim.x) xs[j] = x[j];
  __syncthreads();
  const uint64_t pf = l2_policy_evict_first();
  const int lane = threadIdx.x & 31, warp = threadIdx.x >> 5;
  const int64_t n2 = ncols >> 1;
  const double2 *x2 = reinterpret_cast<const double2 *>(xs);
  int buf = 0;
  for (int64_t row = blockIdx.x; row < nrows; row += gridDim.x, buf ^= 1) {
    const double2 *q2 = reinterpret_cast<const double2 *>(Q + row * ncols);
    double acc0 = 0.0, acc1 = 0.0;
    int64_t j = threadIdx.x;
    for (; j + (U - 1) * (NWARPS * 32) < n2; j += U * NWARPS * 32) {
      double2 a[U];
#pragma unroll
      for (int u = 0; u < U; ++u) a[u] = ld_stream_f64x2(q2 + j + u * NWARPS * 32, pf);
#pragma unroll
      for (int u = 0; u < U; ++u) {
        double2 b = x2[j + u * NWARPS * 32];
        acc0 = fma(a[u].x, b.x, acc0);
        acc1 = fma(a[u].y, b.y, acc1);
      }
    }
    for (; j < n2; j += NWARPS * 32) {
      double2 a = ld_stream_f64x2(q2 + j, pf);
      double2 b = x2[j];
      acc0 = fma(a.x, b.x, acc0);
      acc1 = fma(a.y, b.y, acc1);
    }
    double acc = acc0 + acc1;
#pragma unroll
    for (int s = 16; s > 0; s >>= 1) acc += __shfl_xor_sync(0xffffffffu, acc, s);
    if (lane == 0) part[buf][warp] = acc;
    __syncthreads();
    if (threadIdx.x == 0) {
      double t = 0.0;
#pragma unroll
      for (int w = 0; w < NWARPS; ++w) t += part[buf][w];
      dst[row] = alpha * t;
    }
  }
}

template <int RPB, bool HAS_F2>
__global__ void __launch_bounds__(RPB)
poly_uniform_tile_kernel(const double *__restrict__ V, double *__restrict__ dst, int L,
                         const double *__restrict__ coef, const int32_t *__restrict__ f1,
                         const int32_t *__restrict__ f2, const int32_t *__restrict__ pos,
                         int64_t count, int accumulate) {
  extern __shared__ double prod[];
  const uint64_t pf = l2_policy_evict_first(), pl = l2_policy_evict_last();
  const int64_t ntiles = (count + RPB - 1) / RPB;
  for (int64_t tile = blockIdx.x; tile < ntiles; tile += gridDim.x) {
    const int64_t row0 = tile * RPB;
    const int rows_here = (int)((count - row0) < RPB ? (count - row0) : RPB);
    const int64_t t0 = row0 * (int64_t)L;
    const int nterms = rows_here * L;
    for (int k = threadIdx.x; k < nterms; k += RPB) {
      const int64_t t = t0 + k;
      double v = ld_stream_f64(coef + t, pf) * gather_slot(V, ld_stream_s32(f1 + t, pf), pl);
      if (HAS_F2) v *= gather_slot(V, ld_stream_s32(f2 + t, pf), pl);
      prod[k + (k >> 5)] = v;
    }
    __syncthreads();
    if ((int)threadIdx.x < rows_here) {
      double acc = 0.0;
      const int b = threadIdx.x * L;
      for (int j = 0; j < L; ++j) { int k = b + j; acc += prod[k + (k >> 5)]; }
      const int64_t row = row0 + threadIdx.x;
      const int64_t d = pos ? (int64_t)__ldg(pos + row) : row;
      dst[d] = accumulate ? dst[d] + acc : acc;
    }
    __syncthreads();
  }
}

template <int U, bool HAS_F2>
__global__ void __launch_bounds__(256)
poly1_stream_kernel(const double *__restrict__ V, double *__restrict__ dst, const double *__restrict__ coef,
                    const int32_t *__restrict__ f1, const int32_t *__restrict__ f2,
                    const int32_t *__restrict__ pos, int64_t count, int accumulate) {
  const uint64_t pf = l2_policy_evict_first(), pl = l2_policy_evict_last();
  const int64_t stride = (int64_t)gridDim.x * blockDim.x;
  int64_t k = (int64_t)blockIdx.x * blockDim.x + threadIdx.x;
  for (; k < count; k += U * stride) {
    double c[U];
    int a[U], b[U];
#pragma unroll
    for (int u = 0; u < U; ++u) {
      const int64_t i = k + u * stride;
      const bool ok = i < count;
      c[u] = ok ? ld_stream_f64(coef + i, pf) : 0.0;
      a[u] = ok ? ld_stream_s32(f1 + i, pf) : -1;
      b[u] = (HAS_F2 && ok) ? ld_stream_s32(f2 + i, pf) : -1;
    }
    double v[U];
#pragma unroll
    for (int u = 0; u < U; ++u) {
      v[u] = c[u] * gather_slot(V, a[u], pl);
      if (HAS_F2) v[u] *= gather_slot(V, b[u], pl);
    }
#pragma unroll
    for (int u = 0; u < U; ++u) {
      const int64_t i = k + u * stride;
      if (i < count) {
        const int64_t d = pos ? (int64_t)__ldg(pos + i) : i;
        if (accumulate) dst[d] += v[u]; else st_stream_f64(dst + d, v[u], pf);
      }
    }
  }
}

template <int G, int R, bool HAS_F2, bool UNIFORM>
__global__ void __launch_bounds__(256)
poly_rows_kernel(const double *__restrict__ V, double *__restrict__ dst, const int64_t *__restrict__ ptr,
                 int row_len, const double *__restrict__ coef, const int32_t *__restrict__ f1,
                 const int32_t *__restrict__ f2, const int32_t *__restrict__ pos, int64_t count,
                 int accumulate) {
  const uint64_t pf = l2_policy_evict_first(), pl = l2_policy_evict_last();
  const int lane = threadIdx.x & (G - 1);
  const int64_t group = ((int64_t)blockIdx.x * blockDim.x + threadIdx.x) / G;
  const int64_t ngroups = ((int64_t)gridDim.x * blockDim.x) / G;
  for (int64_t base = group; base < count; base += R * ngroups) {
    int64_t t[R], t1[R];
    double acc[R];
#pragma unroll
    for (int r = 0; r < R; ++r) {
      const int64_t row = base + r * ngroups;
      acc[r] = 0.0;
      if (row < count) {
        if (UNIFORM) { t[r] = row * (int64_t)row_len; t1[r] = t[r] + row_len; }
        else { t[r] = __ldg(ptr + row); t1[r] = __ldg(ptr + row + 1); }
        t[r] += lane;
      } else { t[r] = 0; t1[r] = 0; }
    }
    bool more = true;
    while (more) {
      double c[R];
      int a[R], b[R];
#pragma unroll
      for (int r = 0; r < R; ++r) {
        const bool ok = t[r] < t1[r];
        c[r] = ok ? ld_stream_f64(coef + t[r], pf) : 0.0;
        a[r] = ok ? ld_stream_s32(f1 + t[r], pf) : -1;
        b[r] = (HAS_F2 && ok) ? ld_stream_s32(f2 + t[r], pf) : -1;
      }
      more = false;
#pragma unroll
      for (int r = 0; r < R; ++r) {
        double v = c[r] * gather_slot(V, a[r], pl);
        if (HAS_F2) v *= gather_slot(V, b[r], pl);
        acc[r] += v;
        t[r] += G;
        more |= t[r] < t1[r];
      }
    }
#pragma unroll
    for (int r = 0; r < R; ++r) {
      double v = acc[r];
#pragma unroll
      for (int s = G >> 1; s > 0; s >>= 1) v += __shfl_xor_sync(0xffffffffu, v, s, G);
      const int64_t row = base + r * ngroups;
      if (lane == 0 && row < count) {
        const int64_t d = pos ? (int64_t)__ldg(pos + row) : row;
        dst[d] = accumulate ? dst[d] + v : v;
      }
    }
  }
}

constexpr int FLAT_CHUNK = 256;
constexpr int FLAT_PROD = FLAT_CHUNK + 2 * (FLAT_CHUNK / 16) + 2;
constexpr int FLAT_WARPS = 8;

__device__ __forceinline__ double ld_keep_f64_if(const double *p, bool take, double other, uint64_t pol) {
  double v;
  asm volatile("{\n\t.reg .pred p;\n\tsetp.ne.s32 p, %3, 0;\n\tmov.f64 %0, %4;\n\t"
               "@p ld.global.L2::cache_hint.f64 %0, [%1], %2;\n\t}"
               : "=d"(v) : "l"(p), "l"(pol), "r"((int)take), "d"(other) : "memory");
  return v;
}

__device__ __forceinline__ int2 ld_stream_s32x2(const int2 *p, uint64_t pol) {
  int2 v;
  asm("ld.global.nc.L1::no_allocate.L2::cache_hint.v2.s32 {%0, %1}, [%2], %3;"
      : "=r"(v.x), "=r"(v.y) : "l"(p), "l"(pol));
  return v;
}

template <bool HAS_F2, bool WIN, bool PAD>
__global__ void __launch_bounds__(FLAT_WARPS * 32, 4)
poly_flat_kernel(const double *__restrict__ V, double *dst, const int64_t *__restrict__ ptr, int row_len,
                 const double *__restrict__ coef, const int32_t *__restrict__ f1,
                 const int32_t *__restrict__ f2, const int32_t *__restrict__ pos, int64_t nterms,
                 int accumulate, const int32_t *__restrict__ chunk_row0,
                 const int64_t *__restrict__ chunk_term0, int64_t nchunks, int w0, int W, int pad_shift) {
  __shared__ __align__(16) double prod_all[FLAT_WARPS][FLAT_PROD];
  extern __shared__ __align__(16) double win[];
  if (WIN) {
    for (int j = threadIdx.x; j < W; j += FLAT_WARPS * 32) win[j] = V[w0 + j];
    __syncthreads();
  }
  const uint64_t pf = l2_policy_evict_first(), pl = l2_policy_evict_last();
  auto gather = [&](int idx) -> double {
    if (WIN) {
      const unsigned rel = (unsigned)(idx - w0);
      const bool in = rel < (unsigned)W;
      const double wv = win[in ? rel : 0u];
      const bool out = !in && idx >= 0;
      return ld_keep_f64_if(V + (out ? idx : 0), out, idx < 0 ? 1.0 : wv, pl);
    }
    return ld_keep_f64_if(V + (idx >= 0 ? idx : 0), idx >= 0, 1.0, pl);
  };
  auto padf = [&](int k) -> int { return PAD ? k + ((k >> pad_shift) << 1) : k; };
  auto row_begin = [&](int64_t r) -> int64_t { return ptr ? __ldg(ptr + r) : r * (int64_t)row_len; };
  const int lane = threadIdx.x & 31;
  double *prod = prod_all[threadIdx.x >> 5];
  const int64_t nwarps = (int64_t)gridDim.x * FLAT_WARPS;
  int64_t c = (int64_t)blockIdx.x * FLAT_WARPS + (threadIdx.x >> 5);
  if (c >= nchunks) return;
  int R0 = __ldg(chunk_row0 + c), R1 = __ldg(chunk_row0 + c + 1);
  int64_t a0 = __ldg(chunk_term0 + c);
  while (true) {
    const int64_t cn = c + nwarps;
    int nR0 = 0, nR1 = 0;
    int64_t na0 = 0;
    if (cn < nchunks) { nR0 = __ldg(chunk_row0 + cn); nR1 = __ldg(chunk_row0 + cn + 1); na0 = __ldg(chunk_term0 + cn); }
    int64_t s = 0, e = 0;
    if (R0 + lane < R1) { s = row_begin(R0 + lane); e = row_begin(R0 + lane + 1); }
    if (a0 + FLAT_CHUNK <= nterms) {
      const double2 *c2 = reinterpret_cast<const double2 *>(coef + a0);
      const int2 *a2 = reinterpret_cast<const int2 *>(f1 + a0);
      const int2 *b2 = reinterpret_cast<const int2 *>(f2 + a0);
      double2 cv[4];
      int2 av[4], bv[4];
#pragma unroll
      for (int j = 0; j < 4; ++j) {
        cv[j] = ld_stream_f64x2(c2 + j * 32 + lane, pf);
        av[j] = ld_stream_s32x2(a2 + j * 32 + lane, pf);
        if (HAS_F2) bv[j] = ld_stream_s32x2(b2 + j * 32 + lane, pf);
      }
      double gx[4], gy[4];
#pragma unroll
      for (int j = 0; j < 4; ++j) { gx[j] = gather(av[j].x); gy[j] = gather(av[j].y); }
      if (HAS_F2) {
#pragma unroll
        for (int j = 0; j < 4; ++j) { gx[j] *= gather(bv[j].x); gy[j] *= gather(bv[j].y); }
      }
#pragma unroll
      for (int j = 0; j < 4; ++j) {
        const int q = padf(2 * (j * 32 + lane));
        *reinterpret_cast<double2 *>(prod + q) = make_double2(cv[j].x * gx[j], cv[j].y * gy[j]);
      }
    } else {
      for (int k = lane; k < (int)(nterms - a0); k += 32) {
        double v = ld_stream_f64(coef + a0 + k, pf) * gather(ld_stream_s32(f1 + a0 + k, pf));
        if (HAS_F2) v *= gather(ld_stream_s32(f2 + a0 + k, pf));
        prod[padf(k)] = v;
      }
    }
    __syncwarp();
    for (int r = R0 + lane; r < R1; r += 32) {
      if (r != R0 + lane) { s = row_begin(r); e = row_begin(r + 1); }
      int k = (int)(s - a0);
      const int ke = (int)(e - a0);
      double acc = 0.0;
      for (; k + 4 <= ke; k += 4) {
        const double p0 = prod[padf(k)], p1 = prod[padf(k + 1)], p2 = prod[padf(k + 2)], p3 = prod[padf(k + 3)];
        acc = (((acc + p0) + p1) + p2) + p3;
      }
      for (; k < ke; ++k) acc += prod[padf(k)];
      const int64_t d = pos ? (int64_t)__ldg(pos + r) : r;
      dst[d] = accumulate ? dst[d] + acc : acc;
    }
    if (cn >= nchunks) break;
    c = cn; R0 = nR0; R1 = nR1; a0 = na0;
    __syncwarp();
  }
}

__device__ __forceinline__ double2 ld_pair_if(const double *p, bool take, uint64_t pol) {
  double2 v;
  asm volatile("{\n\t.reg .pred p;\n\tsetp.ne.s32 p, %4, 0;\n\tmov.f64 %0, 0d3FF0000000000000;\n\tmov.f64 %1, 0d0000000000000000;\n\t"
               "@p ld.global.L2::cache_hint.v2.f64 {%0, %1}, [%2], %3;\n\t}"
               : "=d"(v.x), "=d"(v.y) : "l"(p), "l"(pol), "r"((int)take) : "memory");
  return v;
}

template <bool PAD>
__global__ void __launch_bounds__(FLAT_WARPS * 32, 3)
spmvj_flat_kernel(const double *__restrict__ V, double *g, double *__restrict__ jac, const int64_t *__restrict__ ptr,
                  int row_len, const double *__restrict__ coef, const int32_t *__restrict__ f1,
                  const uint8_t *__restrict__ jrank, const int32_t *__restrict__ jsorted,
                  const int32_t *__restrict__ pos, int64_t nterms,
                  const int32_t *__restrict__ chunk_row0, const int64_t *__restrict__ chunk_term0, int64_t nchunks,
                  int pad_shift) {
  __shared__ __align__(16) double prod_all[FLAT_WARPS][FLAT_PROD];
  __shared__ __align__(16) double jbuf_all[FLAT_WARPS][FLAT_CHUNK];
  const uint64_t pf = l2_policy_evict_first(), pl = l2_policy_evict_last();
  auto padf = [&](int k) -> int { return PAD ? k + ((k >> pad_shift) << 1) : k; };
  auto row_begin = [&](int64_t r) -> int64_t { return ptr ? __ldg(ptr + r) : r * (int64_t)row_len; };
  auto pair = [&](int idx) -> double2 { return ld_pair_if(V + (idx >= 0 ? idx : 0), idx >= 0, pl); };
  const int lane = threadIdx.x & 31;
  double *prod = prod_all[threadIdx.x >> 5];
  double *jbuf = jbuf_all[threadIdx.x >> 5];
  const int64_t nwarps = (int64_t)gridDim.x * FLAT_WARPS;
  int64_t c = (int64_t)blockIdx.x * FLAT_WARPS + (threadIdx.x >> 5);
  if (c >= nchunks) return;
  int R0 = __ldg(chunk_row0 + c), R1 = __ldg(chunk_row0 + c + 1);
  int64_t a0 = __ldg(chunk_term0 + c);
  while (true) {
    const int64_t cn = c + nwarps;
    int nR0 = 0, nR1 = 0;
    int64_t na0 = 0;
    if (cn < nchunks) { nR0 = __ldg(chunk_row0 + cn); nR1 = __ldg(chunk_row0 + cn + 1); na0 = __ldg(chunk_term0 + cn); }
    int64_t s = 0, e = 0;
    if (R0 + lane < R1) { s = row_begin(R0 + lane); e = row_begin(R0 + lane + 1); }
    const int64_t own0 = row_begin(R0), own1 = row_begin(R1);
    const int ks = (int)(own0 - a0), ke = (int)(own1 - a0);
    if (a0 + FLAT_CHUNK <= nterms) {
      const double2 *c2 = reinterpret_cast<const double2 *>(coef + a0);
      const int2 *a2 = reinterpret_cast<const int2 *>(f1 + a0);
      const unsigned short *r2 = reinterpret_cast<const unsigned short *>(jrank + a0);
      double2 cv[4];
      int2 av[4];
      unsigned rk[4];
#pragma unroll
      for (int j = 0; j < 4; ++j) {
        cv[j] = ld_stream_f64x2(c2 + j * 32 + lane, pf);
        av[j] = ld_stream_s32x2(a2 + j * 32 + lane, pf);
        rk[j] = __ldg(r2 + j * 32 + lane);
      }
      double2 px[4], py[4];
#pragma unroll
      for (int j = 0; j < 4; ++j) { px[j] = pair(av[j].x); py[j] = pair(av[j].y); }
#pragma unroll
      for (int j = 0; j < 4; ++j) {
        const int k = 2 * (j * 32 + lane);
        *reinterpret_cast<double2 *>(prod + padf(k)) = make_double2(cv[j].x * px[j].x, cv[j].y * py[j].x);
        if (k >= ks && k < ke) jbuf[rk[j] & 0xFF] = cv[j].x * px[j].y;
        if (k + 1 >= ks && k + 1 < ke) jbuf[rk[j] >> 8] = cv[j].y * py[j].y;
      }
    } else {
      for (int k = lane; k < (int)(nterms - a0); k += 32) {
        const double cc = ld_stream_f64(coef + a0 + k, pf);
        const double2 pv = pair(ld_stream_s32(f1 + a0 + k, pf));
        prod[padf(k)] = cc * pv.x;
        if (k >= ks && k < ke) jbuf[jrank[a0 + k]] = cc * pv.y;
      }
    }
    __syncwarp();
    for (int i = lane; i < ke - ks; i += 32) {
      const int q = ld_stream_s32(jsorted + own0 + i, pf);
      if (q >= 0) st_stream_f64(jac + q, jbuf[i], pf);
    }
    for (int r = R0 + lane; r < R1; r += 32) {
      if (r != R0 + lane) { s = row_begin(r); e = row_begin(r + 1); }
      int k = (int)(s - a0);
      const int kend = (int)(e - a0);
      double acc = 0.0;
      for (; k + 4 <= kend; k += 4) {
        const double p0 = prod[padf(k)], p1 = prod[padf(k + 1)], p2 = prod[padf(k + 2)], p3 = prod[padf(k + 3)];
        acc = (((acc + p0) + p1) + p2) + p3;
      }
      for (; k < kend; ++k) acc += prod[padf(k)];
      g[pos ? (int64_t)__ldg(pos + r) : r] = acc;
    }
    if (cn >= nchunks) break;
    c = cn; R0 = nR0; R1 = nR1; a0 = na0;
    __syncwarp();
  }
}

static __global__ void __launch_bounds__(256)
spmvj_rows_kernel(const double *__restrict__ V, double *__restrict__ g, double *__restrict__ jac,
                  const int64_t *__restrict__ ptr, int row_len, const double *__restrict__ coef,
                  const int32_t *__restrict__ f1, const int32_t *__restrict__ qpos, const int32_t *__restrict__ pos,
                  int64_t count) {
  for (int64_t r = (int64_t)blockIdx.x * blockDim.x + threadIdx.x; r < count; r += (int64_t)gridDim.x * blockDim.x) {
    const int64_t t0 = ptr ? ptr[r] : r * (int64_t)row_len, t1 = ptr ? ptr[r + 1] : t0 + row_len;
    double acc = 0.0;
    for (int64_t t = t0; t < t1; ++t) {
      const double c = coef[t];
      const int idx = f1[t], q = qpos[t];
      const double v = idx >= 0 ? V[idx] : 1.0;
      acc += c * v;
      if (q >= 0) jac[q] = c * (idx >= 0 ? V[idx + 1] : 0.0);
    }
    g[pos ? (int64_t)pos[r] : r] = acc;
  }
}

struct ElemDesc {
  int64_t a_off, b_off, count, tile0;
  int64_t dst_off[3];
  double param[3];
  double scale[3];
  int32_t fcode[3];
  int32_t dst_stride[3];
  int32_t nout, a_stride, b_stride;
  int32_t group;
};

enum : int { GRP_NONE = 0, GRP_TRIG = 1, GRP_LOGISTIC = 2, GRP_TANH = 3 };

__host__ __device__ inline int elem_family(int f) {
  if (f == F_SIN || f == F_COS || f == F_NEG_SIN || f == F_NEG_COS) return GRP_TRIG;
  if (f == F_LOGISTIC || f == F_LOGISTIC_D1 || f == F_LOGISTIC_D2) return GRP_LOGISTIC;
  if (f == F_TANH || f == F_TANH_D1 || f == F_TANH_D2) return GRP_TANH;
  return GRP_NONE;
}

template <int GRP>
__device__ __forceinline__ void fused_point(double a, const ElemDesc &d, bool want_val, double (&r)[3]) {
  if constexpr (GRP == GRP_TRIG) {
    double sn, cs;
    sincos(a, &sn, &cs);
#pragma unroll
    for (int o = 0; o < 3; ++o) {
      const int f = d.fcode[o];
      r[o] = f == F_SIN ? sn : (f == F_COS ? cs : (f == F_NEG_SIN ? -sn : -cs));
    }
  } else if constexpr (GRP == GRP_LOGISTIC) {
    const double e = exp(a);
    const double dd = e + 1.0;
    double val = 0.0;
    if (want_val) val = isnan(a) ? a : fmax(a, 0.0) + log1p(a <= 0.0 ? e : 1.0 / e);
#pragma unroll
    for (int o = 0; o < 3; ++o) {
      const int f = d.fcode[o];
      r[o] = f == F_LOGISTIC ? val : (f == F_LOGISTIC_D1 ? e / dd : e / (dd * dd));
    }
  } else {
    const double c = cosh(a);
    const double t = want_val ? tanh(a) : 0.0;
    const double c2 = c * c;
#pragma unroll
    for (int o = 0; o < 3; ++o) {
      const int f = d.fcode[o];
      r[o] = f == F_TANH ? t : (f == F_TANH_D1 ? 1.0 / c2 : -2.0 * (t / c2));
    }
  }
}

template <int GRP>
__device__ __forceinline__ void fused_tile(double *__restrict__ V, const ElemDesc &d, int64_t e0, int64_t e1,
                                           bool vec_ok) {
  const double *__restrict__ A = V + d.a_off;
  bool want_val = false;
  for (int o = 0; o < d.nout; ++o)
    want_val = want_val || d.fcode[o] == F_LOGISTIC || d.fcode[o] == F_TANH || d.fcode[o] == F_TANH_D2;
  if (vec_ok) {
    int64_t k = e0 + 2 * threadIdx.x;
    double2 a = k < e1 ? *reinterpret_cast<const double2 *>(A + k) : make_double2(0.0, 0.0);
    for (; k < e1; k += 512) {
      const double2 an = k + 512 < e1 ? *reinterpret_cast<const double2 *>(A + k + 512) : a;
      double rx[3], ry[3];
      fused_point<GRP>(a.x, d, want_val, rx);
      fused_point<GRP>(a.y, d, want_val, ry);
#pragma unroll
      for (int o = 0; o < 3; ++o)
        if (o < d.nout)
          *reinterpret_cast<double2 *>(V + d.dst_off[o] + k) = make_double2(d.scale[o] * rx[o], d.scale[o] * ry[o]);
      a = an;
    }
  } else {
    const bool pair01 = d.nout >= 2 && d.dst_stride[0] == 2 && d.dst_stride[1] == 2 && d.dst_off[1] == d.dst_off[0] + 1 &&
                        (d.dst_off[0] & 1) == 0;
    for (int64_t k = e0 + threadIdx.x; k < e1; k += 256) {
      double r[3];
      fused_point<GRP>(A[k * d.a_stride], d, want_val, r);
      if (pair01) {
        *reinterpret_cast<double2 *>(V + d.dst_off[0] + 2 * k) = make_double2(d.scale[0] * r[0], d.scale[1] * r[1]);
        if (d.nout > 2) V[d.dst_off[2] + k * d.dst_stride[2]] = d.scale[2] * r[2];
      } else {
#pragma unroll
        for (int o = 0; o < 3; ++o)
          if (o < d.nout) V[d.dst_off[o] + k * d.dst_stride[o]] = d.scale[o] * r[o];
      }
    }
  }
}

constexpr int ELEM_TILE = 2048;

template <int F>
__device__ __forceinline__ void elem_tile(double *__restrict__ V, const ElemDesc &d, int o,
                                          int64_t e0, int64_t e1, bool vec_ok) {
  const double *__restrict__ A = V + d.a_off;
  const double *__restrict__ B = V + d.b_off;
  double *__restrict__ D = V + d.dst_off[o];
  const double p = d.param[o], sc = d.scale[o];
  const int ds = d.dst_stride[o];
  if (vec_ok) {
    int64_t k = e0 + 2 * threadIdx.x;
    const bool bvec = F >= F_REL_ENTR && d.b_stride == 1;
    double2 a = k < e1 ? *reinterpret_cast<const double2 *>(A + k) : make_double2(0.0, 0.0);
    double2 b = make_double2(0.0, 0.0);
    if (F >= F_REL_ENTR) b = bvec ? (k < e1 ? *reinterpret_cast<const double2 *>(B + k) : b) : make_double2(B[0], B[0]);
    for (; k < e1; k += 512) {
      const bool more = k + 512 < e1;
      const double2 an = more ? *reinterpret_cast<const double2 *>(A + k + 512) : a;
      const double2 bn = (bvec && more) ? *reinterpret_cast<const double2 *>(B + k + 512) : b;
      double2 r;
      r.x = sc * apply_fn<F>(a.x, b.x, p);
      r.y = sc * apply_fn<F>(a.y, b.y, p);
      *reinterpret_cast<double2 *>(D + k) = r;
      a = an; b = bn;
    }
  } else {
    for (int64_t k = e0 + threadIdx.x; k < e1; k += 256)
      D[k * ds] = sc * apply_fn<F>(A[k * d.a_stride], F >= F_REL_ENTR ? B[k * d.b_stride] : 0.0, p);
  }
}

static __global__ void __launch_bounds__(256, 3)
elem_batch_kernel(double *__restrict__ V, const ElemDesc *__restrict__ descs, int ndesc, int64_t total_tiles) {
  __shared__ ElemDesc d;
  for (int64_t tile = blockIdx.x; tile < total_tiles; tile += gridDim.x) {
    __syncthreads();
    if (threadIdx.x == 0) {
      int lo = 0, hi = ndesc - 1;
      while (lo < hi) { int mid = (lo + hi + 1) >> 1; if (descs[mid].tile0 <= tile) lo = mid; else hi = mid - 1; }
      d = descs[lo];
    }
    __syncthreads();
    const int64_t e0 = (tile - d.tile0) * ELEM_TILE;
    const int64_t e1 = (e0 + ELEM_TILE < d.count) ? e0 + ELEM_TILE : d.count;
    bool vec_ok = d.a_stride == 1 && (d.a_off & 1) == 0 && (d.b_stride == 0 || (d.b_off & 1) == 0) &&
                  ((e1 - e0) & 1) == 0;
    for (int o = 0; o < d.nout; ++o) vec_ok = vec_ok && (d.dst_off[o] & 1) == 0 && d.dst_stride[o] == 1;
    if (d.group == GRP_TRIG) { fused_tile<GRP_TRIG>(V, d, e0, e1, vec_ok); continue; }
    if (d.group == GRP_LOGISTIC) { fused_tile<GRP_LOGISTIC>(V, d, e0, e1, vec_ok); continue; }
    if (d.group == GRP_TANH) { fused_tile<GRP_TANH>(V, d, e0, e1, vec_ok); continue; }
    for (int o = 0; o < d.nout; ++o) {
      switch (d.fcode[o]) {
#define DNLP_CASE(F) case F: elem_tile<F>(V, d, o, e0, e1, vec_ok); break;
        DNLP_CASE(F_EXP) DNLP_CASE(F_LOG) DNLP_CASE(F_ENTR) DNLP_CASE(F_NEG_LOG_M1) DNLP_CASE(F_RECIP)
        DNLP_CASE(F_NEG_RECIP) DNLP_CASE(F_NEG_RECIP_SQ) DNLP_CASE(F_LOGISTIC) DNLP_CASE(F_LOGISTIC_D1)
        DNLP_CASE(F_LOGISTIC_D2) DNLP_CASE(F_POW) DNLP_CASE(F_SIN) DNLP_CASE(F_COS) DNLP_CASE(F_NEG_SIN)
        DNLP_CASE(F_NEG_COS) DNLP_CASE(F_TAN) DNLP_CASE(F_TAN_D1) DNLP_CASE(F_TAN_D2) DNLP_CASE(F_SINH)
        DNLP_CASE(F_COSH) DNLP_CASE(F_TANH) DNLP_CASE(F_TANH_D1) DNLP_CASE(F_TANH_D2) DNLP_CASE(F_ASINH)
        DNLP_CASE(F_ASINH_D1) DNLP_CASE(F_ASINH_D2) DNLP_CASE(F_ATANH) DNLP_CASE(F_ATANH_D1)
        DNLP_CASE(F_ATANH_D2) DNLP_CASE(F_XEXP) DNLP_CASE(F_XEXP_D1) DNLP_CASE(F_XEXP_D2)
        DNLP_CASE(F_REL_ENTR) DNLP_CASE(F_LOG_RATIO_P1) DNLP_CASE(F_DIV) DNLP_CASE(F_DIV_SQ) DNLP_CASE(F_DIV_CUBE)
#undef DNLP_CASE
        default: break;
      }
    }
  }
}

template <bool HAS_F2>
__global__ void __launch_bounds__(256)
poly_reduce_kernel(const double *__restrict__ V, double *__restrict__ dst, const double *__restrict__ coef,
                   const int32_t *__restrict__ f1, const int32_t *__restrict__ f2, int64_t nterms,
                   int accumulate, double *__restrict__ scratch, unsigned int *__restrict__ ticket) {
  const uint64_t pf = l2_policy_evict_first(), pl = l2_policy_evict_last();
  const int64_t stride = (int64_t)gridDim.x * blockDim.x;
  double acc[4] = {0.0, 0.0, 0.0, 0.0};
  for (int64_t k = (int64_t)blockIdx.x * blockDim.x + threadIdx.x; k < nterms; k += 4 * stride) {
    double c[4];
    int a[4], b[4];
#pragma unroll
    for (int u = 0; u < 4; ++u) {
      const int64_t i = k + u * stride;
      const bool ok = i < nterms;
      c[u] = ok ? ld_stream_f64(coef + i, pf) : 0.0;
      a[u] = ok ? ld_stream_s32(f1 + i, pf) : -1;
      b[u] = (HAS_F2 && ok) ? ld_stream_s32(f2 + i, pf) : -1;
    }
#pragma unroll
    for (int u = 0; u < 4; ++u) {
      double v = c[u] * gather_slot(V, a[u], pl);
      if (HAS_F2) v *= gather_slot(V, b[u], pl);
      acc[u] += v;
    }
  }
  double v = (acc[0] + acc[1]) + (acc[2] + acc[3]);
#pragma unroll
  for (int s = 16; s > 0; s >>= 1) v += __shfl_xor_sync(0xffffffffu, v, s);
  __shared__ double wsum[8];
  __shared__ bool last;
  const int lane = threadIdx.x & 31, warp = threadIdx.x >> 5;
  if (lane == 0) wsum[warp] = v;
  __syncthreads();
  if (threadIdx.x == 0) {
    double t = 0.0;
#pragma unroll
    for (int w = 0; w < 8; ++w) t += wsum[w];
    scratch[blockIdx.x] = t;
    __threadfence();
    last = atomicAdd(ticket, 1u) == gridDim.x - 1;
  }
  __syncthreads();
  if (last && warp == 0) {
    __threadfence();
    double t = 0.0;
    for (int i = lane; i < (int)gridDim.x; i += 32) t += __ldcg(scratch + i);
#pragma unroll
    for (int s = 16; s > 0; s >>= 1) t += __shfl_xor_sync(0xffffffffu, t, s);
    if (lane == 0) {
      dst[0] = accumulate ? dst[0] + t : t;
      *ticket = 0;
    }
  }
}

static __global__ void __launch_bounds__(256)
gather_kernel(const double *__restrict__ src, const int32_t *__restrict__ pos, double *__restrict__ dst,
              int64_t count) {
  for (int64_t k = (int64_t)blockIdx.x * blockDim.x + threadIdx.x; k < count; k += (int64_t)gridDim.x * blockDim.x)
    dst[k] = src[pos[k]];
}

template <bool HAS_F2>
__global__ void __launch_bounds__(256)
sum_range_kernel(const double *__restrict__ V, double *__restrict__ dst, int64_t s0, int64_t s1, int64_t n,
                 double c, int accumulate, double *__restrict__ scratch, unsigned int *__restrict__ ticket) {
  const int64_t stride = (int64_t)gridDim.x * blockDim.x;
  double acc[4] = {0.0, 0.0, 0.0, 0.0};
  for (int64_t k = (int64_t)blockIdx.x * blockDim.x + threadIdx.x; k < n; k += 4 * stride) {
#pragma unroll
    for (int u = 0; u < 4; ++u) {
      const int64_t i = k + u * stride;
      if (i < n) acc[u] += HAS_F2 ? V[s0 + i] * V[s1 + i] : V[s0 + i];
    }
  }
  double v = (acc[0] + acc[1]) + (acc[2] + acc[3]);
#pragma unroll
  for (int s = 16; s > 0; s >>= 1) v += __shfl_xor_sync(0xffffffffu, v, s);
  __shared__ double wsum[8];
  __shared__ bool last;
  const int lane = threadIdx.x & 31, warp = threadIdx.x >> 5;
  if (lane == 0) wsum[warp] = v;
  __syncthreads();
  if (threadIdx.x == 0) {
    double t = 0.0;
#pragma unroll
    for (int w = 0; w < 8; ++w) t += wsum[w];
    scratch[blockIdx.x] = t;
    __threadfence();
    last = atomicAdd(ticket, 1u) == gridDim.x - 1;
  }
  __syncthreads();
  if (last && warp == 0) {
    __threadfence();
    double t = 0.0;
    for (int i = lane; i < (int)gridDim.x; i += 32) t += __ldcg(scratch + i);
#pragma unroll
    for (int s = 16; s > 0; s >>= 1) t += __shfl_xor_sync(0xffffffffu, t, s);
    if (lane == 0) {
      dst[0] = accumulate ? dst[0] + c * t : c * t;
      *ticket = 0;
    }
  }
}

template <bool HAS_F2>
__global__ void __launch_bounds__(256)
poly1_contig_kernel(const double *__restrict__ V, double *__restrict__ dst, const double *__restrict__ coef,
                    int64_t s0, int64_t s1, int64_t count) {
  const uint64_t pf = l2_policy_evict_first();
  for (int64_t k = (int64_t)blockIdx.x * blockDim.x + threadIdx.x; k < count; k += (int64_t)gridDim.x * blockDim.x) {
    double v = ld_stream_f64(coef + k, pf) * V[s0 + k];
    if (HAS_F2) v *= V[s1 + k];
    st_stream_f64(dst + k, v, pf);
  }
}

}
```

include/dnlp_b200.h:

```cpp
#ifndef DNLP_B200_H
#define DNLP_B200_H

#include <stdint.h>

#ifdef __cplusplus
extern "C" {
#endif

typedef struct dnlp_oracle dnlp_oracle;

enum { DNLP_ELEM = 1, DNLP_POLY = 2, DNLP_GEMV = 3, DNLP_SCALE = 4, DNLP_SPMVJ = 5 };
enum { DNLP_DST_V = 0, DNLP_DST_F = 1, DNLP_DST_GRAD = 2, DNLP_DST_G = 3, DNLP_DST_JAC = 4, DNLP_DST_HESS = 5 };
enum { DNLP_PROG_F = 0, DNLP_PROG_GRAD = 1, DNLP_PROG_G = 2, DNLP_PROG_JAC = 3, DNLP_PROG_HESS = 4,
       DNLP_PROG_ALL = 5, DNLP_NPROG = 6 };

typedef struct {
  int32_t kind;
  int32_t dst_space;
  int64_t dst_off;
  int64_t count;
  int32_t fcode;
  int32_t a_stride;
  int32_t b_stride;
  int32_t accumulate;
  double param;
  int64_t a_off;
  int64_t b_off;
  const int64_t *ptr;
  const double *coef;
  const int32_t *f1;
  const int32_t *f2;
  const int32_t *pos;
  int64_t nterms;
  int32_t row_len;
  int32_t uses_lam;
  int32_t level;
  int32_t dep_mask;
  const double *Q;
  int64_t ncols;
  int64_t x_off;
  double alpha;
  int64_t s_slot;
  const int32_t *deps;
  int64_t n_deps;
  int32_t dst_stride;
  int32_t reserved0;
  double post_scale;
  const int32_t *qpos;
} dnlp_instr_desc;

typedef struct {
  int64_t n;
  int64_t m;
  int64_t nslots;
  int64_t nnz_jac;
  int64_t nnz_hess;
  int32_t n_instr;
  const dnlp_instr_desc *instrs;
  const int32_t *prog[DNLP_NPROG];
  int32_t prog_len[DNLP_NPROG];
  double f_const;
  const double *grad_const;
  const double *g_const;
  const double *jac_const;
  const double *hess_const;
  int64_t n_params;
  const double *params;
} dnlp_tape_desc;

int dnlp_device_count(void);
const char *dnlp_version(void);
int dnlp_device_synchronize(int device);

int dnlp_create(const dnlp_tape_desc *tape, int device, dnlp_oracle **out);
void dnlp_destroy(dnlp_oracle *o);
const char *dnlp_last_error(dnlp_oracle *o);

int dnlp_eval_f(dnlp_oracle *o, const double *x, double *f);
int dnlp_eval_grad(dnlp_oracle *o, const double *x, double *grad );
int dnlp_eval_g(dnlp_oracle *o, const double *x, double *g );
int dnlp_eval_jac(dnlp_oracle *o, const double *x, double *vals );
int dnlp_eval_hess(dnlp_oracle *o, const double *x, const double *lam , double sigma,
                   double *vals );
int dnlp_eval_all(dnlp_oracle *o, const double *x, const double *lam, double sigma,
                  double *f, double *grad, double *g, double *jac, double *hess);

int dnlp_set_params(dnlp_oracle *o, const double *values, int64_t count);

int dnlp_set_dynamic(dnlp_oracle *o, int32_t dst_space, const int32_t *pos, int64_t count);
int dnlp_eval_dyn(dnlp_oracle *o, int32_t prog, const double *x, const double *lam, double sigma,
                  double *compact);

int dnlp_bind_outputs(dnlp_oracle *o, double *f, double *grad, double *g, double *jac, int32_t eager);

int dnlp_run(dnlp_oracle *o, int32_t prog, const double *x, const double *lam, double sigma);
void *dnlp_output_ptr(dnlp_oracle *o, int32_t dst_space);

void *dnlp_host_alloc(int64_t bytes);
void dnlp_host_free(void *p);

int dnlp_upload_point(dnlp_oracle *o, const double *x, const double *lam, double sigma);
int dnlp_run_device(dnlp_oracle *o, int32_t prog_mask, int32_t iters, float *elapsed_ms);
int dnlp_profile_instrs(dnlp_oracle *o, int32_t prog, int32_t iters, float *ms_per_instr );
int dnlp_read_output(dnlp_oracle *o, int32_t dst_space, double *out);
int64_t dnlp_kernel_launches(dnlp_oracle *o);
const char *dnlp_instr_kernel(dnlp_oracle *o, int32_t instr);
int dnlp_set_cache(dnlp_oracle *o, int32_t enabled);
int dnlp_set_graphs(dnlp_oracle *o, int32_t enabled);
int dnlp_set_parallel(dnlp_oracle *o, int32_t enabled);
int dnlp_set_windows(dnlp_oracle *o, int32_t enabled);

typedef struct dnlp_batch dnlp_batch;
int dnlp_batch_create(const dnlp_tape_desc *tape, int device, int32_t batch, dnlp_batch **out);
void dnlp_batch_destroy(dnlp_batch *b);
const char *dnlp_batch_last_error(dnlp_batch *b);
int dnlp_batch_eval(dnlp_batch *b, const double *X, const double *LAM, const double *SIGMA,
                    double *F, double *GRAD, double *G, double *JAC, double *HESS);
int dnlp_batch_upload(dnlp_batch *b, const double *X, const double *LAM, const double *SIGMA);
int dnlp_batch_run_device(dnlp_batch *b, int32_t prog_mask, int32_t iters, float *elapsed_ms);
int dnlp_batch_read_output(dnlp_batch *b, int32_t dst_space, double *out);
int dnlp_batch_profile_instrs(dnlp_batch *b, int32_t prog, int32_t iters, float *ms_per_instr);
int dnlp_batch_profile_groups(dnlp_batch *b, int32_t iters, float *ms_per_group, double *flops_per_group,
                              int32_t max_groups);
int64_t dnlp_batch_kernel_launches(dnlp_batch *b);

int dnlp_batch_kkt_setup(dnlp_batch *b, int64_t ns, const int32_t *slack_rows, const int32_t *jac_rows,
                         const int32_t *jac_cols, const int32_t *hess_rows, const int32_t *hess_cols);
int dnlp_batch_kkt_solve(dnlp_batch *b, int32_t count, const int32_t *starts, const double *sigma, const double *dw,
                         const double *dc, const double *rhs, double *sol, int32_t *inertia, double *wquad,
                         float *elapsed_ms);
int dnlp_batch_kkt_matrix(dnlp_batch *b, int32_t start, double *out);

typedef struct dnlp_comm dnlp_comm;
typedef struct dnlp_shard dnlp_shard;
int dnlp_comm_unique_id(char *out128);
int dnlp_comm_create(const char *nccl_id , int rank, int world, int device,
                     dnlp_comm **out);
void dnlp_comm_destroy(dnlp_comm *c);
const char *dnlp_comm_last_error(dnlp_comm *c);
int dnlp_comm_has_nccl(dnlp_comm *c);
int dnlp_comm_ipc_handle(dnlp_comm *c, char *out64);
int dnlp_comm_open_peers(dnlp_comm *c, const char *handles );
int dnlp_comm_allreduce_host(dnlp_comm *c, double *vec, int64_t count);

int dnlp_shard_create(dnlp_oracle *local, dnlp_comm *comm, int root, dnlp_shard **out);
void dnlp_shard_destroy(dnlp_shard *s);
const char *dnlp_shard_last_error(dnlp_shard *s);
int dnlp_shard_set_output(dnlp_shard *s, int32_t dst_space, int64_t n_shared_total, const int32_t *shared_src,
                          const int32_t *shared_global_pos, int64_t n_owned, const int32_t *owned_pos,
                          const int32_t *owned_global_pos, int64_t global_len, const double *global_const,
                          int64_t n_dyn, const int32_t *dyn_global_pos);
int dnlp_shard_root_handles(dnlp_shard *s, char *out384);
int dnlp_shard_open_root(dnlp_shard *s, const char *handles384);
int dnlp_shard_set_layout(dnlp_shard *s, int32_t n_xruns, const int64_t *xsrc, const int64_t *xlen,
                          int32_t n_lruns, const int64_t *lsrc, const int64_t *llen);
int dnlp_shard_eval(dnlp_shard *s, int32_t prog, const double *x_local, const double *lam_local, double sigma,
                    double *host_out );
int dnlp_shard_run_device(dnlp_shard *s, int32_t prog_mask, int32_t iters, float *elapsed_ms);

int dnlp_shard_share_control(dnlp_shard *s, const char *shm_name, int32_t create);
int dnlp_shard_share_output(dnlp_shard *s, int32_t dst_space, const char *shm_name, int32_t create, int64_t n_runs,
                            const int64_t *local_start, const int64_t *global_start, const int64_t *length,
                            double **host_array);
int dnlp_shard_share_unlink(const char *shm_name);
int dnlp_shard_share_reset(dnlp_shard *s);
int dnlp_shard_share_inputs(dnlp_shard *s, const char *shm_x, const char *shm_lam, int32_t create, int64_t n_global,
                            int64_t m_global, double **x_host, double **lam_host);
int dnlp_shard_post_command(dnlp_shard *s, int32_t prog, const double *x, const double *lam, double sigma,
                            int32_t force, int32_t *flags);
int dnlp_shard_wait_command(dnlp_shard *s, double timeout_s, int32_t *prog, double *sigma, int32_t *flags);
int dnlp_shard_share_release(double *host_array, int64_t count);

#ifdef __cplusplus
}
#endif
#endif
```

Before: 6752.

## Fold output polynomials into batched elementwise kernel sinks and skip unread stores

Adds a host-side fold planner that detects output POLY instructions (gradient/Jacobian rows or the scalar objective sum) whose terms are contiguous runs of batched elementwise results. The batched elementwise kernel then writes those contributions directly to output spaces or reduces them into the objective through per-tile partials and a ticket counter. Elementwise intermediates that nothing else reads are not stored. This removes separate POLY launches and round-trips through the value buffer, but adds dependency tracking, residual instructions and cache-validity changes that make scheduling more complex.

```diff
diff --git a/dnlp_b200/_cabi.py b/dnlp_b200/_cabi.py
--- a/dnlp_b200/_cabi.py
+++ b/dnlp_b200/_cabi.py
@@ -3,6 +3,7 @@
 
 import numpy as np
 
+from . import fold
 from . import tape as T
 
 _PKG = os.path.dirname(os.path.abspath(__file__))
@@ -43,11 +44,25 @@
     ]
 
 
+class FoldSeg(C.Structure):
+    _fields_ = [
+        ("poly", C.c_int32), ("elem", C.c_int32), ("k0", C.c_int64), ("len", C.c_int64), ("out_off", C.c_int64),
+        ("coef", C.c_double), ("f2_slot", C.c_int64), ("f2_stride", C.c_int32), ("reserved", C.c_int32),
+    ]
+
+
+class FoldResid(C.Structure):
+    _fields_ = [
+        ("poly", C.c_int32), ("reserved", C.c_int32), ("nterms", C.c_int64),
+        ("coef", c_f64p), ("f1", c_i32p), ("f2", c_i32p), ("pos", c_i32p),
+    ]
+
+
 EXPORTS = [
     "dnlp_device_count", "dnlp_version", "dnlp_device_synchronize", "dnlp_create", "dnlp_destroy", "dnlp_last_error",
     "dnlp_eval_f", "dnlp_eval_grad", "dnlp_eval_g", "dnlp_eval_jac", "dnlp_eval_hess", "dnlp_eval_all",
     "dnlp_host_alloc", "dnlp_host_free", "dnlp_upload_point", "dnlp_run_device", "dnlp_profile_instrs",
-    "dnlp_read_output", "dnlp_kernel_launches", "dnlp_set_cache", "dnlp_set_graphs", "dnlp_set_parallel", "dnlp_set_windows", "dnlp_set_dynamic", "dnlp_eval_dyn", "dnlp_bind_outputs", "dnlp_set_params", "dnlp_instr_kernel", "dnlp_run", "dnlp_output_ptr",
+    "dnlp_read_output", "dnlp_kernel_launches", "dnlp_set_cache", "dnlp_set_graphs", "dnlp_set_parallel", "dnlp_set_windows", "dnlp_set_dynamic", "dnlp_eval_dyn", "dnlp_bind_outputs", "dnlp_set_params", "dnlp_instr_kernel", "dnlp_run", "dnlp_output_ptr", "dnlp_set_fold_plan",
     "dnlp_batch_create", "dnlp_batch_destroy", "dnlp_batch_last_error", "dnlp_batch_eval", "dnlp_batch_upload",
     "dnlp_batch_run_device", "dnlp_batch_read_output", "dnlp_batch_profile_instrs", "dnlp_batch_kernel_launches", "dnlp_batch_profile_groups",
     "dnlp_batch_kkt_setup", "dnlp_batch_kkt_solve", "dnlp_batch_kkt_matrix",
@@ -109,6 +124,8 @@
     L.dnlp_bind_outputs.argtypes = [vp, c_f64p, c_f64p, c_f64p, c_f64p, C.c_int32]
     L.dnlp_set_dynamic.argtypes = [vp, C.c_int32, c_i32p, C.c_int64]
     L.dnlp_eval_dyn.argtypes = [vp, C.c_int32, c_f64p, c_f64p, C.c_double, c_f64p]
+    L.dnlp_set_fold_plan.argtypes = [vp, C.POINTER(C.c_uint8), C.c_int32, C.POINTER(FoldSeg), C.c_int32,
+                                     C.POINTER(FoldResid)]
     L.dnlp_batch_create.argtypes = [C.POINTER(TapeDesc), C.c_int, C.c_int32, C.POINTER(vp)]
     L.dnlp_batch_destroy.argtypes = [vp]
     L.dnlp_batch_destroy.restype = None
@@ -320,6 +337,26 @@
             raise RuntimeError("dnlp_create failed: %s" % L.dnlp_last_error(None).decode())
         self.h = h
         self._L = L
+        self.set_fold_plan(fold.plan(tape))
+
+    def set_fold_plan(self, plan):
+        segs = [s for poly in sorted(plan.segments) for s in plan.segments[poly]]
+        if not segs:
+            return
+        sa = (FoldSeg * len(segs))()
+        for d, s in zip(sa, segs):
+            d.poly, d.elem, d.k0, d.len, d.out_off = s.poly, s.elem, s.k0, s.length, s.out_off
+            d.coef, d.f2_slot, d.f2_stride = s.coef, s.f2, s.f2_stride
+        keep = []
+        ra = (FoldResid * max(len(plan.residual), 1))()
+        for d, poly in zip(ra, sorted(plan.residual)):
+            coef, f1, f2, pos = plan.residual[poly]
+            keep += [coef, f1, f2, pos]
+            d.poly, d.nterms = poly, int(coef.size)
+            d.coef, d.f1, d.f2, d.pos = _p(coef, c_f64p), _p(f1, c_i32p), _p(f2, c_i32p), _p(pos, c_i32p)
+        stored = np.ascontiguousarray(plan.stored, dtype=np.uint8)
+        self.check(self._L.dnlp_set_fold_plan(self.h, stored.ctypes.data_as(C.POINTER(C.c_uint8)), len(segs), sa,
+                                              len(plan.residual), ra))
 
     def check(self, rc):
         if rc != 0:
diff --git a/dnlp_b200/csrc/dnlp_cabi.cu b/dnlp_b200/csrc/dnlp_cabi.cu
--- a/dnlp_b200/csrc/dnlp_cabi.cu
+++ b/dnlp_b200/csrc/dnlp_cabi.cu
@@ -245,21 +245,50 @@
 }
 
 int dnlp_oracle::build_batches() {
+  for (int bi = 0; bi < 2 * DNLP_NPROG; ++bi) batch[bi] = ElemBatch();
   for (int bi = 0; bi < 2 * DNLP_NPROG; ++bi) {
     const int p = bi >> 1;
     const bool want_short = (bi & 1) != 0;
     ElemBatch &B = batch[bi];
+    auto batchable = [&](const dnlp_instr_desc &d) {
+      return d.kind == DNLP_ELEM && d.level == 0 && !d.uses_lam && d.dst_space == DNLP_DST_V && d.count > 0;
+    };
+    std::vector<int32_t> folded;
+    std::unordered_map<int32_t, std::vector<const dnlp_fold_seg *>> segs_of;
+    for (int32_t id : prog[p])
+      if (instrs[id].fold) folded.push_back(id);
+    for (const dnlp_fold_seg &sg : fold_segs)
+      if (std::find(folded.begin(), folded.end(), sg.poly) != folded.end()) segs_of[sg.elem].push_back(&sg);
+    auto same_source = [](const dnlp_instr_desc &x, const dnlp_instr_desc &y) {
+      return x.a_off == y.a_off && x.b_off == y.b_off && x.count == y.count && x.a_stride == y.a_stride &&
+             x.b_stride == y.b_stride;
+    };
+    auto feeds_reduction = [&](const dnlp_instr_desc &d) {
+      for (int32_t id : prog[p]) {
+        const dnlp_instr_desc &e = instrs[id].d;
+        if (!batchable(e) || !same_source(e, d)) continue;
+        auto it = segs_of.find(id);
+        if (it != segs_of.end())
+          for (const dnlp_fold_seg *sg : it->second) if (sg->out_off < 0) return true;
+      }
+      return false;
+    };
     std::vector<dnlp::ElemDesc> descs;
+    std::vector<std::vector<int32_t>> outs_of;
     for (int32_t id : prog[p]) {
       const dnlp_instr_desc &d = instrs[id].d;
-      if (d.kind != DNLP_ELEM || d.level != 0 || d.uses_lam || d.dst_space != DNLP_DST_V || d.count <= 0) continue;
-      if ((d.count < batch_split) != want_short) continue;
+      if (!batchable(d)) continue;
+      if ((d.count < batch_split && !feeds_reduction(d)) != want_short) continue;
       bool merged = false;
-      for (auto &e : descs) {
+      for (size_t q = 0; q < descs.size(); ++q) {
+        dnlp::ElemDesc &e = descs[q];
         if (e.nout < 3 && e.a_off == d.a_off && e.b_off == d.b_off && e.count == d.count &&
             e.a_stride == d.a_stride && e.b_stride == d.b_stride) {
           e.fcode[e.nout] = d.fcode; e.param[e.nout] = d.param; e.dst_off[e.nout] = d.dst_off;
-          e.dst_stride[e.nout] = d.dst_stride > 0 ? d.dst_stride : 1; e.scale[e.nout] = d.post_scale; ++e.nout;
+          e.dst_stride[e.nout] = d.dst_stride > 0 ? d.dst_stride : 1; e.scale[e.nout] = d.post_scale;
+          if (instrs[id].stored) e.vstore |= 1 << e.nout;
+          ++e.nout;
+          outs_of[q].push_back(id);
           merged = true;
           break;
         }
@@ -269,12 +298,51 @@
         e.a_off = d.a_off; e.b_off = d.b_off; e.count = d.count; e.a_stride = d.a_stride; e.b_stride = d.b_stride;
         e.nout = 1; e.fcode[0] = d.fcode; e.param[0] = d.param; e.dst_off[0] = d.dst_off;
         e.dst_stride[0] = d.dst_stride > 0 ? d.dst_stride : 1; e.scale[0] = d.post_scale;
+        e.vstore = instrs[id].stored ? 1 : 0;
         for (int k = 1; k < 3; ++k) { e.dst_stride[k] = 1; e.scale[k] = 1.0; }
         descs.push_back(e);
+        outs_of.push_back({id});
       }
       B.members.push_back(id);
-    }
-    if (B.members.size() < 2) { B.members.clear(); continue; }
+      if (instrs[id].stored) B.stores = true;
+    }
+    std::vector<dnlp::ElemSink> sinks;
+    int32_t red_poly = -1;
+    for (size_t q = 0; q < descs.size(); ++q) {
+      dnlp::ElemDesc &e = descs[q];
+      e.sink0 = (int32_t)sinks.size();
+      for (int o = 0; o < e.nout; ++o) {
+        auto it = segs_of.find(outs_of[q][o]);
+        if (it == segs_of.end()) continue;
+        for (const dnlp_fold_seg *sg : it->second) {
+          const dnlp_instr_desc &P = instrs[sg->poly].d;
+          dnlp::ElemSink k{};
+          k.e0 = sg->k0; k.e1 = sg->k0 + sg->len; k.coef = sg->coef; k.out = o;
+          k.f2 = sg->f2_slot >= 0 ? V + sg->f2_slot : nullptr;
+          k.f2_stride = sg->f2_stride;
+          if (sg->out_off < 0) {
+            if (red_poly >= 0 && red_poly != sg->poly) { err = "fold plan: two folded reductions in one program"; return 1; }
+            red_poly = sg->poly;
+            k.sum = 1;
+          } else {
+            k.dst = out[P.dst_space] + sg->out_off;
+          }
+          sinks.push_back(k);
+          B.out_mask |= 1 << P.dst_space;
+        }
+      }
+      e.nsink = (int32_t)sinks.size() - e.sink0;
+      if (e.nsink > dnlp::ELEM_MAX_SINKS) { err = "fold plan: too many folded segments on one elementwise source"; return 1; }
+    }
+    const bool lead = want_short && !B.members.empty() && batch[bi - 1].nsink > 0;
+    if (sinks.empty() && B.members.size() < 2 && !lead) { B = ElemBatch(); continue; }
+    for (int32_t id : folded)
+      if (instrs[id].fold == 1) {
+        bool here = false;
+        for (const dnlp_fold_seg &sg : fold_segs)
+          if (sg.poly == id && std::find(B.members.begin(), B.members.end(), sg.elem) != B.members.end()) here = true;
+        if (here) B.members.push_back(id);
+      }
     for (auto &e : descs) {
       e.group = dnlp::GRP_NONE;
       if (e.nout < 2 || !fuse_enabled) continue;
@@ -287,18 +355,32 @@
     for (auto &e : descs) { e.tile0 = tiles; tiles += (e.count + dnlp::ELEM_TILE - 1) / dnlp::ELEM_TILE; }
     B.ndesc = (int)descs.size();
     B.total_tiles = tiles;
+    B.nsink = (int)sinks.size();
     if (upload(descs.data(), (int64_t)descs.size(), &B.descs)) return 1;
+    if (!sinks.empty() && upload(sinks.data(), (int64_t)sinks.size(), &B.sinks)) return 1;
+    if (red_poly >= 0) {
+      const dnlp_instr_desc &P = instrs[red_poly].d;
+      B.red = out[P.dst_space] + P.dst_off;
+      void *q = nullptr;
+      CK(cudaMalloc(&q, (size_t)(tiles + 2) * sizeof(double)));
+      owned.push_back(q);
+      B.partial = static_cast<double *>(q);
+      CK(cudaMalloc(&q, 16 * sizeof(unsigned int)));
+      owned.push_back(q);
+      B.ticket = static_cast<unsigned int *>(q);
+      CK(cudaMemset(B.ticket, 0, 16 * sizeof(unsigned int)));
+    }
   }
   return 0;
 }
 
 int dnlp_oracle::launch_node(int32_t node) {
-  if (node >= 0) return launch(instrs[node]);
+  if (node >= 0) return launch(instrs[node].resid >= 0 ? resid_instrs[instrs[node].resid] : instrs[node]);
   ElemBatch &B = batch[-node - 1];
   if (cur == nullptr) { cur = stream; cur_lane = 0; }
   int64_t cap = (int64_t)sm_count * 8;
   int grid = (int)(B.total_tiles < cap ? B.total_tiles : cap);
-  dnlp::elem_batch_kernel<<<grid, 256, 0, cur>>>(V, B.descs, B.ndesc, B.total_tiles);
+  dnlp::elem_batch_kernel<<<grid, 256, 0, cur>>>(V, B.descs, B.ndesc, B.total_tiles, B.sinks, B.red, B.partial, B.ticket);
   ++launches;
   cudaError_t e = cudaPeekAtLastError();
   if (e != cudaSuccess) { err = std::string("kernel launch failed: ") + cudaGetErrorString(e); return 1; }
@@ -324,10 +406,6 @@
   const size_t N = nodes.size();
   if (N < 2 || !parallel_enabled) return issue_serial(nodes);
   std::unordered_map<int32_t, int> producer;
-  for (size_t k = 0; k < N; ++k) {
-    if (nodes[k] >= 0) producer[nodes[k]] = (int)k;
-    else for (int32_t id : batch[-nodes[k] - 1].members) producer[id] = (int)k;
-  }
   std::vector<int> lane_of(N, 0);
   int last_on_lane[NLANE];
   bool joined[NLANE];
@@ -354,6 +432,15 @@
         if (last_writer[DNLP_DST_JAC] >= 0) deps.push_back(last_writer[DNLP_DST_JAC]);
         last_writer[DNLP_DST_JAC] = (int)k;
       }
+    } else {
+      const ElemBatch &B = batch[-nodes[k] - 1];
+      for (int s = 1; s < 6; ++s)
+        if ((B.out_mask >> s) & 1) {
+          if (last_writer[s] >= 0) deps.push_back(last_writer[s]);
+          last_writer[s] = (int)k;
+        }
+      if (B.nsink > 0 && B.stores && k > 0)
+        for (int l = 0; l < NLANE; ++l) if (last_on_lane[l] >= 0) deps.push_back(last_on_lane[l]);
     }
     int L = -1;
     if (nodes[k] >= 0 && big_serial_terms > 0 && instrs[nodes[k]].d.kind != DNLP_ELEM &&
@@ -373,6 +460,8 @@
     CK(cudaEventRecord(done, lane[L]));
     lane_of[k] = L;
     last_on_lane[L] = (int)k;
+    if (nodes[k] >= 0) producer[nodes[k]] = (int)k;
+    else for (int32_t id : batch[-nodes[k] - 1].members) producer[id] = (int)k;
   }
   for (int l = 1; l < NLANE; ++l)
     if (joined[l] && last_on_lane[l] >= 0) CK(cudaStreamWaitEvent(stream, event_at(1 + (size_t)last_on_lane[l]), 0));
@@ -389,7 +478,7 @@
     for (int bi = 2 * p + 1; bi >= 2 * p; --bi) {
       ElemBatch &B = batch[bi];
       bool use_batch = !B.members.empty();
-      if (use_batch) for (int32_t id : B.members) if (done[id]) { use_batch = false; break; }
+      if (use_batch && B.nsink == 0) for (int32_t id : B.members) if (done[id]) { use_batch = false; break; }
       if (use_batch) {
         nodes.push_back(-(bi + 1));
         key = (key ^ (uint64_t)(0x10000 + bi)) * 1099511628211ull;
@@ -405,7 +494,8 @@
       key = (key ^ (uint64_t)(id + 1)) * 1099511628211ull;
       if (keep) done[id] = 1;
     }
-    for (auto &f : done) if (f == 2) f = 1;
+    for (size_t i = 0; i < done.size(); ++i)
+      if (done[i] == 2) done[i] = instrs[i].stored && !instrs[i].fold ? 1 : 0;
   }
   if (nodes.empty()) return 0;
 
@@ -440,7 +530,10 @@
   } else if (issue_serial(nodes)) return 1;
 
   for (int32_t nd : nodes) {
-    if (nd < 0) { for (int32_t id : batch[-nd - 1].members) valid[id] = 1; continue; }
+    if (nd < 0) {
+      for (int32_t id : batch[-nd - 1].members) if (instrs[id].stored && cacheable(instrs[id])) valid[id] = 1;
+      continue;
+    }
     if (cacheable(instrs[nd])) valid[nd] = 1;
   }
   return 0;
@@ -921,6 +1014,62 @@
   return 0;
 }
 
+int dnlp_set_fold_plan(dnlp_oracle *o, const uint8_t *stored, int32_t n_seg, const dnlp_fold_seg *segs,
+                       int32_t n_resid, const dnlp_fold_resid *resid) {
+  ENTER(o);
+  CK(cudaStreamSynchronize(o->stream));
+  const int64_t ni = (int64_t)o->instrs.size();
+  if (!o->fold_segs.empty() || !o->resid_instrs.empty()) { err = "fold plan already set"; return 1; }
+  for (int32_t q = 0; q < n_seg; ++q) {
+    const dnlp_fold_seg &sg = segs[q];
+    if (sg.poly < 0 || sg.poly >= ni || sg.elem < 0 || sg.elem >= ni) { err = "fold plan: unknown instruction"; return 1; }
+    const dnlp_instr_desc &P = o->instrs[sg.poly].d, &E = o->instrs[sg.elem].d;
+    if (P.kind != DNLP_POLY || P.dst_space == DNLP_DST_V || P.accumulate || E.kind != DNLP_ELEM || E.level != 0 ||
+        E.uses_lam || E.dst_space != DNLP_DST_V || E.dst_stride != 1)
+      { err = "fold plan: segment does not join a batched ELEM to an output POLY"; return 1; }
+    if (sg.len <= 0 || sg.k0 < 0 || sg.k0 + sg.len > E.count) { err = "fold plan: segment outside its ELEM"; return 1; }
+    if (sg.out_off < 0 ? P.count != 1 : sg.out_off + sg.len > o->out_len[P.dst_space])
+      { err = "fold plan: segment outside its output"; return 1; }
+    if (sg.f2_slot >= 0 && (sg.f2_stride < 0 || sg.f2_stride > 1 || sg.f2_slot + (sg.len - 1) * sg.f2_stride >= o->nslots))
+      { err = "fold plan: bad second factor"; return 1; }
+    o->fold_segs.push_back(sg);
+    o->instrs[sg.poly].fold = 1;
+  }
+  for (int32_t q = 0; q < n_resid; ++q) {
+    const dnlp_fold_resid &r = resid[q];
+    if (r.poly < 0 || r.poly >= ni || !o->instrs[r.poly].fold || r.nterms <= 0 || !r.coef || !r.f1 || !r.pos)
+      { err = "fold plan: bad residual"; return 1; }
+    const DevInstr &src = o->instrs[r.poly];
+    for (int64_t t = 0; t < r.nterms; ++t)
+      if (r.pos[t] < 0 || src.d.dst_off + r.pos[t] >= o->out_len[src.d.dst_space] || r.f1[t] >= o->nslots ||
+          (r.f2 && r.f2[t] >= o->nslots)) { err = "fold plan: residual index out of range"; return 1; }
+    DevInstr D;
+    D.d = src.d;
+    D.d.count = r.nterms; D.d.nterms = r.nterms; D.d.ptr = nullptr; D.d.row_len = 1; D.d.accumulate = 0;
+    D.d.f2 = nullptr;
+    D.deps = src.deps;
+    if (o->upload(r.coef, r.nterms, const_cast<double **>(&D.d.coef))) return 1;
+    if (o->upload(r.f1, r.nterms, const_cast<int32_t **>(&D.d.f1))) return 1;
+    if (r.f2 && o->upload(r.f2, r.nterms, const_cast<int32_t **>(&D.d.f2))) return 1;
+    if (o->upload(r.pos, r.nterms, const_cast<int32_t **>(&D.d.pos))) return 1;
+    D.has_f2 = r.f2 != nullptr;
+    o->instrs[r.poly].fold = 2;
+    o->instrs[r.poly].resid = (int)o->resid_instrs.size();
+    o->resid_instrs.push_back(D);
+  }
+  for (int64_t i = 0; i < ni; ++i) {
+    DevInstr &I = o->instrs[i];
+    I.stored = !stored || stored[i] != 0;
+    if (!I.stored && I.d.kind != DNLP_ELEM) { err = "fold plan: only an ELEM result can go unstored"; return 1; }
+  }
+  if (o->build_batches()) return 1;
+  for (auto &kv : o->graphs) if (kv.second.exec) cudaGraphExecDestroy(kv.second.exec);
+  o->graphs.clear();
+  std::fill(o->valid.begin(), o->valid.end(), 0);
+  CK(cudaStreamSynchronize(o->stream));
+  return 0;
+}
+
 int dnlp_set_params(dnlp_oracle *o, const double *values, int64_t count) {
   ENTER(o);
   if (count != o->n_params) { err = "wrong number of parameter values"; return 1; }
diff --git a/dnlp_b200/csrc/dnlp_engine.h b/dnlp_b200/csrc/dnlp_engine.h
--- a/dnlp_b200/csrc/dnlp_engine.h
+++ b/dnlp_b200/csrc/dnlp_engine.h
@@ -42,6 +42,9 @@
   int pad_shift = 31;
   uint8_t *jrank = nullptr;
   int32_t *jsorted = nullptr;
+  int fold = 0;
+  int resid = -1;
+  bool stored = true;
 };
 
 struct ElemBatch {
@@ -49,6 +52,13 @@
   int ndesc = 0;
   int64_t total_tiles = 0;
   std::vector<int32_t> members;
+  dnlp::ElemSink *sinks = nullptr;
+  int nsink = 0;
+  int out_mask = 0;
+  bool stores = false;
+  double *red = nullptr;
+  double *partial = nullptr;
+  unsigned int *ticket = nullptr;
 };
 
 }
@@ -64,6 +74,8 @@
   double *out[6] = {nullptr, nullptr, nullptr, nullptr, nullptr, nullptr};
   int64_t out_len[6] = {0, 0, 0, 0, 0, 0};
   std::vector<DevInstr> instrs;
+  std::vector<DevInstr> resid_instrs;
+  std::vector<dnlp_fold_seg> fold_segs;
   std::vector<int32_t> prog[DNLP_NPROG];
   ElemBatch batch[2 * DNLP_NPROG];
   int64_t batch_split = 1 << 16;
diff --git a/dnlp_b200/csrc/dnlp_kernels.cuh b/dnlp_b200/csrc/dnlp_kernels.cuh
--- a/dnlp_b200/csrc/dnlp_kernels.cuh
+++ b/dnlp_b200/csrc/dnlp_kernels.cuh
@@ -712,7 +712,51 @@
   int32_t dst_stride[3];
   int32_t nout, a_stride, b_stride;
   int32_t group;
+  int32_t vstore;
+  int32_t sink0, nsink;
+  int32_t pad0;
 };
+
+struct ElemSink {
+  int64_t e0, e1;
+  double *dst;
+  const double *f2;
+  double coef;
+  int32_t out, sum, f2_stride, pad0;
+};
+constexpr int ELEM_MAX_SINKS = 16;
+
+__device__ __forceinline__ double pick3(const double (&r)[3], int o) { return o == 0 ? r[0] : (o == 1 ? r[1] : r[2]); }
+
+__device__ __forceinline__ void sink_one(const ElemSink &q, int64_t k, double v, double &facc) {
+  if (k < q.e0 || k >= q.e1) return;
+  if (q.sum) { facc += q.coef * v; return; }
+  double r = q.coef * v;
+  if (q.f2) r *= q.f2[(k - q.e0) * q.f2_stride];
+  __stcs(q.dst + (k - q.e0), r);
+}
+
+__device__ __forceinline__ void sink_pair(const ElemSink &q, int64_t k, double vx, double vy, double &facc) {
+  const bool ix = k >= q.e0 && k < q.e1, iy = k + 1 >= q.e0 && k + 1 < q.e1;
+  if (!ix && !iy) return;
+  if (q.sum) {
+    if (ix) facc += q.coef * vx;
+    if (iy) facc += q.coef * vy;
+    return;
+  }
+  double rx = q.coef * vx, ry = q.coef * vy;
+  if (q.f2) {
+    if (ix) rx *= q.f2[(k - q.e0) * q.f2_stride];
+    if (iy) ry *= q.f2[(k + 1 - q.e0) * q.f2_stride];
+  }
+  double *p = q.dst + (k - q.e0);
+  if (ix && iy && (reinterpret_cast<uintptr_t>(p) & 15) == 0) {
+    __stcs(reinterpret_cast<double2 *>(p), make_double2(rx, ry));
+  } else {
+    if (ix) __stcs(p, rx);
+    if (iy) __stcs(p + 1, ry);
+  }
+}
 
 enum : int { GRP_NONE = 0, GRP_TRIG = 1, GRP_LOGISTIC = 2, GRP_TANH = 3 };
 
@@ -756,8 +800,8 @@
 }
 
 template <int GRP>
-__device__ __forceinline__ void fused_tile(double *__restrict__ V, const ElemDesc &d, int64_t e0, int64_t e1,
-                                           bool vec_ok) {
+__device__ __forceinline__ void fused_tile(double *__restrict__ V, const ElemDesc &d, const ElemSink *sk,
+                                           int64_t e0, int64_t e1, bool vec_ok, double &facc) {
   const double *__restrict__ A = V + d.a_off;
   bool want_val = false;
   for (int o = 0; o < d.nout; ++o)
@@ -771,25 +815,32 @@
       fused_point<GRP>(a.x, d, want_val, rx);
       fused_point<GRP>(a.y, d, want_val, ry);
 #pragma unroll
-      for (int o = 0; o < 3; ++o)
-        if (o < d.nout)
-          *reinterpret_cast<double2 *>(V + d.dst_off[o] + k) = make_double2(d.scale[o] * rx[o], d.scale[o] * ry[o]);
+      for (int o = 0; o < 3; ++o) {
+        rx[o] = d.scale[o] * rx[o];
+        ry[o] = d.scale[o] * ry[o];
+        if (o < d.nout && ((d.vstore >> o) & 1))
+          *reinterpret_cast<double2 *>(V + d.dst_off[o] + k) = make_double2(rx[o], ry[o]);
+      }
+      for (int s = 0; s < d.nsink; ++s) sink_pair(sk[s], k, pick3(rx, sk[s].out), pick3(ry, sk[s].out), facc);
       a = an;
     }
   } else {
     const bool pair01 = d.nout >= 2 && d.dst_stride[0] == 2 && d.dst_stride[1] == 2 && d.dst_off[1] == d.dst_off[0] + 1 &&
-                        (d.dst_off[0] & 1) == 0;
+                        (d.dst_off[0] & 1) == 0 && (d.vstore & 3) == 3;
     for (int64_t k = e0 + threadIdx.x; k < e1; k += 256) {
       double r[3];
       fused_point<GRP>(A[k * d.a_stride], d, want_val, r);
+#pragma unroll
+      for (int o = 0; o < 3; ++o) r[o] = d.scale[o] * r[o];
       if (pair01) {
-        *reinterpret_cast<double2 *>(V + d.dst_off[0] + 2 * k) = make_double2(d.scale[0] * r[0], d.scale[1] * r[1]);
-        if (d.nout > 2) V[d.dst_off[2] + k * d.dst_stride[2]] = d.scale[2] * r[2];
+        *reinterpret_cast<double2 *>(V + d.dst_off[0] + 2 * k) = make_double2(r[0], r[1]);
+        if (d.nout > 2 && ((d.vstore >> 2) & 1)) V[d.dst_off[2] + k * d.dst_stride[2]] = r[2];
       } else {
 #pragma unroll
         for (int o = 0; o < 3; ++o)
-          if (o < d.nout) V[d.dst_off[o] + k * d.dst_stride[o]] = d.scale[o] * r[o];
-      }
+          if (o < d.nout && ((d.vstore >> o) & 1)) V[d.dst_off[o] + k * d.dst_stride[o]] = r[o];
+      }
+      for (int s = 0; s < d.nsink; ++s) sink_one(sk[s], k, pick3(r, sk[s].out), facc);
     }
   }
 }
@@ -797,13 +848,14 @@
 constexpr int ELEM_TILE = 2048;
 
 template <int F>
-__device__ __forceinline__ void elem_tile(double *__restrict__ V, const ElemDesc &d, int o,
-                                          int64_t e0, int64_t e1, bool vec_ok) {
+__device__ __forceinline__ void elem_tile(double *__restrict__ V, const ElemDesc &d, const ElemSink *sk, int o,
+                                          int64_t e0, int64_t e1, bool vec_ok, double &facc) {
   const double *__restrict__ A = V + d.a_off;
   const double *__restrict__ B = V + d.b_off;
   double *__restrict__ D = V + d.dst_off[o];
   const double p = d.param[o], sc = d.scale[o];
   const int ds = d.dst_stride[o];
+  const bool store = (d.vstore >> o) & 1;
   if (vec_ok) {
     int64_t k = e0 + 2 * threadIdx.x;
     const bool bvec = F >= F_REL_ENTR && d.b_stride == 1;
@@ -817,18 +869,28 @@
       double2 r;
       r.x = sc * apply_fn<F>(a.x, b.x, p);
       r.y = sc * apply_fn<F>(a.y, b.y, p);
-      *reinterpret_cast<double2 *>(D + k) = r;
+      if (store) *reinterpret_cast<double2 *>(D + k) = r;
+      for (int s = 0; s < d.nsink; ++s)
+        if (sk[s].out == o) sink_pair(sk[s], k, r.x, r.y, facc);
       a = an; b = bn;
     }
   } else {
-    for (int64_t k = e0 + threadIdx.x; k < e1; k += 256)
-      D[k * ds] = sc * apply_fn<F>(A[k * d.a_stride], F >= F_REL_ENTR ? B[k * d.b_stride] : 0.0, p);
+    for (int64_t k = e0 + threadIdx.x; k < e1; k += 256) {
+      const double r = sc * apply_fn<F>(A[k * d.a_stride], F >= F_REL_ENTR ? B[k * d.b_stride] : 0.0, p);
+      if (store) D[k * ds] = r;
+      for (int s = 0; s < d.nsink; ++s)
+        if (sk[s].out == o) sink_one(sk[s], k, r, facc);
+    }
   }
 }
 
 static __global__ void __launch_bounds__(256, 3)
-elem_batch_kernel(double *__restrict__ V, const ElemDesc *__restrict__ descs, int ndesc, int64_t total_tiles) {
+elem_batch_kernel(double *__restrict__ V, const ElemDesc *__restrict__ descs, int ndesc, int64_t total_tiles,
+                  const ElemSink *__restrict__ sinks, double *red, double *__restrict__ partial,
+                  unsigned int *__restrict__ ticket) {
   __shared__ ElemDesc d;
+  __shared__ ElemSink sk[ELEM_MAX_SINKS];
+  __shared__ double wsum[8];
   for (int64_t tile = blockIdx.x; tile < total_tiles; tile += gridDim.x) {
     __syncthreads();
     if (threadIdx.x == 0) {
@@ -837,28 +899,65 @@
       d = descs[lo];
     }
     __syncthreads();
+    if ((int)threadIdx.x < d.nsink) sk[threadIdx.x] = sinks[d.sink0 + threadIdx.x];
+    if (d.nsink > 0) __syncthreads();
     const int64_t e0 = (tile - d.tile0) * ELEM_TILE;
     const int64_t e1 = (e0 + ELEM_TILE < d.count) ? e0 + ELEM_TILE : d.count;
     bool vec_ok = d.a_stride == 1 && (d.a_off & 1) == 0 && (d.b_stride == 0 || (d.b_off & 1) == 0) &&
                   ((e1 - e0) & 1) == 0;
     for (int o = 0; o < d.nout; ++o) vec_ok = vec_ok && (d.dst_off[o] & 1) == 0 && d.dst_stride[o] == 1;
-    if (d.group == GRP_TRIG) { fused_tile<GRP_TRIG>(V, d, e0, e1, vec_ok); continue; }
-    if (d.group == GRP_LOGISTIC) { fused_tile<GRP_LOGISTIC>(V, d, e0, e1, vec_ok); continue; }
-    if (d.group == GRP_TANH) { fused_tile<GRP_TANH>(V, d, e0, e1, vec_ok); continue; }
-    for (int o = 0; o < d.nout; ++o) {
-      switch (d.fcode[o]) {
-#define DNLP_CASE(F) case F: elem_tile<F>(V, d, o, e0, e1, vec_ok); break;
-        DNLP_CASE(F_EXP) DNLP_CASE(F_LOG) DNLP_CASE(F_ENTR) DNLP_CASE(F_NEG_LOG_M1) DNLP_CASE(F_RECIP)
-        DNLP_CASE(F_NEG_RECIP) DNLP_CASE(F_NEG_RECIP_SQ) DNLP_CASE(F_LOGISTIC) DNLP_CASE(F_LOGISTIC_D1)
-        DNLP_CASE(F_LOGISTIC_D2) DNLP_CASE(F_POW) DNLP_CASE(F_SIN) DNLP_CASE(F_COS) DNLP_CASE(F_NEG_SIN)
-        DNLP_CASE(F_NEG_COS) DNLP_CASE(F_TAN) DNLP_CASE(F_TAN_D1) DNLP_CASE(F_TAN_D2) DNLP_CASE(F_SINH)
-        DNLP_CASE(F_COSH) DNLP_CASE(F_TANH) DNLP_CASE(F_TANH_D1) DNLP_CASE(F_TANH_D2) DNLP_CASE(F_ASINH)
-        DNLP_CASE(F_ASINH_D1) DNLP_CASE(F_ASINH_D2) DNLP_CASE(F_ATANH) DNLP_CASE(F_ATANH_D1)
-        DNLP_CASE(F_ATANH_D2) DNLP_CASE(F_XEXP) DNLP_CASE(F_XEXP_D1) DNLP_CASE(F_XEXP_D2)
-        DNLP_CASE(F_REL_ENTR) DNLP_CASE(F_LOG_RATIO_P1) DNLP_CASE(F_DIV) DNLP_CASE(F_DIV_SQ) DNLP_CASE(F_DIV_CUBE)
+    double facc = 0.0;
+    if (d.group == GRP_TRIG) fused_tile<GRP_TRIG>(V, d, sk, e0, e1, vec_ok, facc);
+    else if (d.group == GRP_LOGISTIC) fused_tile<GRP_LOGISTIC>(V, d, sk, e0, e1, vec_ok, facc);
+    else if (d.group == GRP_TANH) fused_tile<GRP_TANH>(V, d, sk, e0, e1, vec_ok, facc);
+    else {
+      for (int o = 0; o < d.nout; ++o) {
+        switch (d.fcode[o]) {
+#define DNLP_CASE(F) case F: elem_tile<F>(V, d, sk, o, e0, e1, vec_ok, facc); break;
+          DNLP_CASE(F_EXP) DNLP_CASE(F_LOG) DNLP_CASE(F_ENTR) DNLP_CASE(F_NEG_LOG_M1) DNLP_CASE(F_RECIP)
+          DNLP_CASE(F_NEG_RECIP) DNLP_CASE(F_NEG_RECIP_SQ) DNLP_CASE(F_LOGISTIC) DNLP_CASE(F_LOGISTIC_D1)
+          DNLP_CASE(F_LOGISTIC_D2) DNLP_CASE(F_POW) DNLP_CASE(F_SIN) DNLP_CASE(F_COS) DNLP_CASE(F_NEG_SIN)
+          DNLP_CASE(F_NEG_COS) DNLP_CASE(F_TAN) DNLP_CASE(F_TAN_D1) DNLP_CASE(F_TAN_D2) DNLP_CASE(F_SINH)
+          DNLP_CASE(F_COSH) DNLP_CASE(F_TANH) DNLP_CASE(F_TANH_D1) DNLP_CASE(F_TANH_D2) DNLP_CASE(F_ASINH)
+          DNLP_CASE(F_ASINH_D1) DNLP_CASE(F_ASINH_D2) DNLP_CASE(F_ATANH) DNLP_CASE(F_ATANH_D1)
+          DNLP_CASE(F_ATANH_D2) DNLP_CASE(F_XEXP) DNLP_CASE(F_XEXP_D1) DNLP_CASE(F_XEXP_D2)
+          DNLP_CASE(F_REL_ENTR) DNLP_CASE(F_LOG_RATIO_P1) DNLP_CASE(F_DIV) DNLP_CASE(F_DIV_SQ) DNLP_CASE(F_DIV_CUBE)
 #undef DNLP_CASE
-        default: break;
-      }
+          default: break;
+        }
+      }
+    }
+    if (red) {
+#pragma unroll
+      for (int s = 16; s > 0; s >>= 1) facc += __shfl_xor_sync(0xffffffffu, facc, s);
+      if ((threadIdx.x & 31) == 0) wsum[threadIdx.x >> 5] = facc;
+      __syncthreads();
+      if (threadIdx.x == 0) {
+        double t = 0.0;
+#pragma unroll
+        for (int w = 0; w < 8; ++w) t += wsum[w];
+        partial[tile] = t;
+      }
+    }
+  }
+  if (!red) return;
+  __shared__ bool last;
+  __syncthreads();
+  if (threadIdx.x == 0) {
+    __threadfence();
+    last = atomicAdd(ticket, 1u) == gridDim.x - 1;
+  }
+  __syncthreads();
+  if (last && threadIdx.x < 32) {
+    __threadfence();
+    const int lane = threadIdx.x;
+    double t = 0.0;
+    for (int64_t i = lane; i < total_tiles; i += 32) t += __ldcg(partial + i);
+#pragma unroll
+    for (int s = 16; s > 0; s >>= 1) t += __shfl_xor_sync(0xffffffffu, t, s);
+    if (lane == 0) {
+      *red = t;
+      *ticket = 0;
     }
   }
 }
diff --git a/dnlp_b200/fold.py b/dnlp_b200/fold.py
--- /dev/null
+++ b/dnlp_b200/fold.py
@@ -0,0 +1,210 @@
+import numpy as np
+
+from . import tape as T
+
+MAX_SINKS_PER_ELEM = 5
+MAX_SEGMENTS_PER_POLY = 64
+MIN_SEGMENT_TERMS = 2
+
+
+class Segment:
+    __slots__ = ("poly", "elem", "t0", "k0", "length", "coef", "out_off", "f2", "f2_stride")
+
+    def __init__(self, **kw):
+        for k, v in kw.items():
+            setattr(self, k, v)
+
+    def __repr__(self):
+        return ("Segment(poly=%d, elem=%d, t0=%d, k0=%d, length=%d, coef=%r, out_off=%d, f2=%d, f2_stride=%d)"
+                % (self.poly, self.elem, self.t0, self.k0, self.length, self.coef, self.out_off, self.f2,
+                   self.f2_stride))
+
+
+class FoldPlan:
+
+    def __init__(self, tape):
+        self.tape = tape
+        self.segments = {}
+        self.residual = {}
+        self.stored = np.ones(len(tape.instrs), dtype=bool)
+
+    def folded(self, poly):
+        return poly in self.segments
+
+    def fully_folded(self, poly):
+        return poly in self.segments and poly not in self.residual
+
+    def __bool__(self):
+        return bool(self.segments)
+
+
+def batchable(ins):
+    return (ins.kind == T.K_ELEM and ins.level == 0 and not ins.uses_lam and ins.dst_space == T.DST_V
+            and ins.count > 0 and ins.dst_stride == 1)
+
+
+def _one_term_rows(ins):
+    lens = np.diff(ins.ptr)
+    return lens.size == ins.count and bool(np.all(lens == 1))
+
+
+def _runs(ins, elem_of, tmp):
+    f1 = np.asarray(ins.f1, dtype=np.int64)
+    nt = f1.size
+    if nt == 0:
+        return []
+    ok = f1 >= 0
+    e = np.full(nt, -1, dtype=np.int64)
+    e[ok] = elem_of[f1[ok]]
+    ok &= e >= 0
+    f2 = None if ins.f2 is None else np.asarray(ins.f2, dtype=np.int64)
+    if f2 is not None:
+        ok &= f2 < tmp
+    brk = np.ones(nt, dtype=bool)
+    if nt > 1:
+        same = (e[1:] == e[:-1]) & (f1[1:] == f1[:-1] + 1) & (ins.coef[1:] == ins.coef[:-1])
+        if ins.pos is not None:
+            pos = np.asarray(ins.pos, dtype=np.int64)
+            same &= pos[1:] == pos[:-1] + 1
+        if f2 is not None:
+            none = f2 < 0
+            d = f2[1:] - f2[:-1]
+            same &= (none[1:] & none[:-1]) | (~none[1:] & ~none[:-1] & ((d == 0) | (d == 1)))
+        brk[1:] = ~same
+    brk |= ~ok
+    starts = np.flatnonzero(brk & ok)
+    if starts.size > MAX_SEGMENTS_PER_POLY:
+        return None
+    nxt = np.flatnonzero(brk)
+    out = []
+    for s in starts:
+        i = np.searchsorted(nxt, s, side="right")
+        t1 = int(nxt[i]) if i < nxt.size else nt
+        s = int(s)
+        while f2 is not None and f2[s] >= 0 and t1 - s > 2:
+            d = np.diff(f2[s:t1])
+            bad = np.flatnonzero(d != d[0])
+            if bad.size == 0:
+                break
+            cut = s + int(bad[0]) + 1
+            out.append((s, cut))
+            s = cut
+            if len(out) > MAX_SEGMENTS_PER_POLY:
+                return None
+        out.append((s, t1))
+    return out
+
+
+def plan(tape):
+    P = FoldPlan(tape)
+    instrs = tape.instrs
+    tmp = tape.tmp_slot
+    in_prog = {}
+    for name, ids in tape.programs.items():
+        for i in ids:
+            in_prog.setdefault(int(i), set()).add(name)
+    elem_of = np.full(tape.nslots, -1, dtype=np.int64)
+    slot0 = {}
+    for ins in instrs:
+        if batchable(ins):
+            elem_of[ins.dst_off:ins.dst_off + ins.count] = ins.id
+            slot0[ins.id] = int(ins.dst_off)
+    nsinks = {}
+    for ins in instrs:
+        if ins.kind != T.K_POLY or ins.dst_space == T.DST_V or ins.accumulate or ins.dep_mask == T.DEP_SIGMA:
+            continue
+        reduction = ins.count == 1 and ins.dst_space == T.DST_F
+        if not reduction and not _one_term_rows(ins):
+            continue
+        runs = _runs(ins, elem_of, tmp)
+        if not runs:
+            continue
+        progs = in_prog.get(ins.id, set())
+        segs = []
+        for t0, t1 in runs:
+            if t1 - t0 < MIN_SEGMENT_TERMS:
+                continue
+            el = int(elem_of[ins.f1[t0]])
+            if any(el not in in_prog or p not in in_prog[el] for p in progs):
+                continue
+            has_f2 = ins.f2 is not None and ins.f2[t0] >= 0
+            if reduction and has_f2:
+                continue
+            stride = 0
+            if has_f2 and t1 - t0 > 1:
+                stride = int(ins.f2[t0 + 1] - ins.f2[t0])
+            out_off = -1
+            if not reduction:
+                out_off = int(ins.dst_off) + (int(ins.pos[t0]) if ins.pos is not None else t0)
+            segs.append(Segment(poly=ins.id, elem=el, t0=t0, k0=int(ins.f1[t0]) - slot0[el], length=t1 - t0,
+                                coef=float(ins.coef[t0]), out_off=out_off,
+                                f2=int(ins.f2[t0]) if has_f2 else -1, f2_stride=stride))
+        if reduction and sum(s.length for s in segs) != ins.coef.size:
+            continue
+        need = {}
+        for s in segs:
+            need[s.elem] = need.get(s.elem, 0) + 1
+        if any(nsinks.get(el, 0) + c > MAX_SINKS_PER_ELEM for el, c in need.items()):
+            if reduction:
+                continue
+            kept, used = [], dict(nsinks)
+            for s in segs:
+                if used.get(s.elem, 0) < MAX_SINKS_PER_ELEM:
+                    used[s.elem] = used.get(s.elem, 0) + 1
+                    kept.append(s)
+            segs = kept
+        if not segs:
+            continue
+        for s in segs:
+            nsinks[s.elem] = nsinks.get(s.elem, 0) + 1
+        P.segments[ins.id] = segs
+        covered = np.zeros(ins.coef.size, dtype=bool)
+        for s in segs:
+            covered[s.t0:s.t0 + s.length] = True
+        if not covered.all():
+            keep = np.flatnonzero(~covered)
+            f2 = None
+            if ins.f2 is not None and np.any(ins.f2[keep] >= 0):
+                f2 = np.ascontiguousarray(ins.f2[keep], dtype=np.int32)
+            pos = ins.pos[keep] if ins.pos is not None else keep
+            P.residual[ins.id] = (np.ascontiguousarray(ins.coef[keep], dtype=np.float64),
+                                  np.ascontiguousarray(ins.f1[keep], dtype=np.int32), f2,
+                                  np.ascontiguousarray(pos, dtype=np.int32))
+    read = np.zeros(tape.nslots + 2, dtype=bool)
+
+    def mark(idx):
+        idx = np.asarray(idx, dtype=np.int64)
+        read[idx[idx >= 0]] = True
+
+    for ins in instrs:
+        if ins.kind in (T.K_POLY, T.K_SPMVJ):
+            if ins.id in P.segments:
+                if ins.id in P.residual:
+                    coef, f1, f2, pos = P.residual[ins.id]
+                    mark(f1)
+                    if f2 is not None:
+                        mark(f2)
+                for s in P.segments[ins.id]:
+                    if s.f2 >= 0:
+                        mark(s.f2 + s.f2_stride * np.arange(s.length))
+                continue
+            mark(ins.f1)
+            if ins.f2 is not None:
+                mark(ins.f2)
+            if ins.kind == T.K_SPMVJ:
+                f1 = np.asarray(ins.f1, dtype=np.int64)
+                mark(f1[f1 >= 0] + 1)
+        elif ins.kind == T.K_ELEM:
+            k = np.arange(ins.count, dtype=np.int64)
+            mark(ins.a_off + k * ins.a_stride)
+            mark(ins.b_off + k * ins.b_stride)
+        elif ins.kind == T.K_GEMV:
+            read[ins.x_off:ins.x_off + ins.ncols] = True
+        elif ins.kind == T.K_SCALE:
+            read[ins.s_slot] = True
+    folded_elems = {s.elem for segs in P.segments.values() for s in segs}
+    for el in folded_elems:
+        ins = instrs[el]
+        if not read[ins.dst_off:ins.dst_off + ins.count].any():
+            P.stored[el] = False
+    return P
diff --git a/include/dnlp_b200.h b/include/dnlp_b200.h
--- a/include/dnlp_b200.h
+++ b/include/dnlp_b200.h
@@ -96,6 +96,31 @@
 int dnlp_run(dnlp_oracle *o, int32_t prog, const double *x, const double *lam, double sigma);
 void *dnlp_output_ptr(dnlp_oracle *o, int32_t dst_space);
 
+typedef struct {
+  int32_t poly;
+  int32_t elem;
+  int64_t k0;
+  int64_t len;
+  int64_t out_off;
+  double coef;
+  int64_t f2_slot;
+  int32_t f2_stride;
+  int32_t reserved;
+} dnlp_fold_seg;
+
+typedef struct {
+  int32_t poly;
+  int32_t reserved;
+  int64_t nterms;
+  const double *coef;
+  const int32_t *f1;
+  const int32_t *f2;
+  const int32_t *pos;
+} dnlp_fold_resid;
+
+int dnlp_set_fold_plan(dnlp_oracle *o, const uint8_t *stored , int32_t n_seg, const dnlp_fold_seg *segs,
+                       int32_t n_resid, const dnlp_fold_resid *resid);
+
 void *dnlp_host_alloc(int64_t bytes);
 void dnlp_host_free(void *p);
 
```

Result: slower. 6531, median of 6 (-3.3%).
